# polli-labs/linnaeus

Measured on AMD Instinct MI355X. Metric: images/sec (train fwd+bwd) mFormerV1_sm 3x224x224, higher is better.
Workload: dtype bf16; 1 GPU; mFormerV1_sm train step (forward + 4-task CE loss + backward + AdamW (one HIP launch)), bf16 operands / fp32 accumulate+residual, batch 256/GPU, 3x224x224 synthetic, DropPath 0.2, gradient checkpointing off; per_gpu_batch=256, global_batch=256, parallelism=dp1, grad_mode=direct

## Files before the change

include/lnx.h:

```cpp
#ifndef LNX_H
#define LNX_H
#include <stdint.h>

#ifdef __cplusplus
extern "C" {
#endif

#define LNX_F32 0
#define LNX_BF16 1

const char* lnx_last_error(void);
int lnx_version(void);
int lnx_device_cus(void);
int lnx_set_cu_margin(int cus);

typedef struct lnx_rowmap {
    int group, pad, off;
} lnx_rowmap;

enum { LNX_ACT_NONE = 0, LNX_ACT_GELU = 1, LNX_ACT_RELU = 2, LNX_ACT_GELU_BWD = 3, LNX_ACT_RELU_BWD = 4,
       LNX_ACT_GELU_D = 5, LNX_ACT_MUL_AUX = 6 };
enum { LNX_ADDR_PLAIN = 0, LNX_ADDR_PATCH2 = 1 };

typedef struct lnx_gemm_args {
    int dtype;
    int M, N, K;
    const void* A;
    int64_t lda;
    const void* W;
    int64_t ldw;
    void* C;
    int64_t ldc;
    int out_f32;
    int a_mode, Hin, Win, Cin;
    int c_mode;
    lnx_rowmap c_map;
    const float* bias;
    void* c2;
    int64_t ldc2;
    int act;
    const void* aux;
    int64_t ldaux;
    const float* gamma;
    const float* rowscale;
    int rows_per_sample;
    const float* res;
    int64_t ldres;
    void* c8;
    int64_t ldc8;
    void* c8_scales;
} lnx_gemm_args;

int lnx_gemm_nt(const lnx_gemm_args* args, void* stream);

#define LNX_GEMM_GROUP_MAX 8
int lnx_gemm_nt_group_ok(const lnx_gemm_args* problems, int n, int accumulate);
int lnx_gemm_nt_group(const lnx_gemm_args* problems, int n, int accumulate, void* stream);

enum { LNX_NT_KERNEL_NONE = 0, LNX_NT_KERNEL_V1 = 1 , LNX_NT_KERNEL_V2 = 2 ,
       LNX_NT_KERNEL_SKINNY = 3 , LNX_NT_KERNEL_V4 = 4 ,
       LNX_NT_KERNEL_FP8 = 6 , LNX_NT_KERNEL_V7 = 7 ,
       LNX_NT_KERNEL_MX8 = 8 , LNX_NT_KERNEL_V9 = 9 ,
       LNX_NT_KERNEL_EXPERIMENT = 15 , LNX_NT_KERNEL_KINDS = 16 };
int lnx_last_nt_kernel(void);
int64_t lnx_nt_kernel_launches(int kind);
int lnx_nt_dispatch(const lnx_gemm_args* args);

int lnx_amax(const void* x, int x_dtype, int64_t ldx, int rows, int cols, float* amax, void* stream);
int lnx_quantize_fp8(const void* x, int x_dtype, int64_t ldx, int rows, int cols, const float* amax, void* y, int64_t ldy, float* scale_out, void* stream);
int lnx_gemm_nt_fp8(const lnx_gemm_args* args, const float* a_scale, const float* w_scale, void* stream);

int lnx_quantize_mxfp8(const void* x, int x_dtype, int64_t ldx, int rows, int cols, void* y, int64_t ldy, void* scales, void* stream);
int lnx_gemm_nt_mxfp8(const lnx_gemm_args* args, const void* a_scales, const void* w_scales, void* stream);

typedef struct lnx_wgrad_args {
    int dtype;
    int M, N, K;
    const void* dY;
    int64_t lddy;
    const void* A;
    int64_t lda;
    int a_mode, Hin, Win, Cin;
    float* dW;
    int64_t lddw;
    int k_perm_c;
    float* db;
    int splits;
    int k_store;
    float* ws;
    int64_t ws_floats;
    int defer;
} lnx_wgrad_args;
#define LNX_TN_WS_FLOATS (256 * (256 * 128 + 256))

int lnx_gemm_tn(const lnx_wgrad_args* args, void* stream);
int lnx_gemm_tn_flush(void* stream);
int lnx_gemm_tn_discard(void);


typedef struct lnx_ln_args {
    int M, C;
    float eps;
    const void* x;
    int x_dtype;
    int64_t ldx;
    lnx_rowmap x_map;
    const float* w;
    const float* b;
    void* y;
    int y_dtype;
    int64_t ldy;
    lnx_rowmap y_map;
    const void* add;
    int64_t ldadd;
    float* mean;
    float* rstd;
    void* y8;
    int64_t ldy8;
    void* y8_scales;
} lnx_ln_args;
int lnx_layernorm_fwd(const lnx_ln_args* args, void* stream);

typedef struct lnx_ln_bwd_args {
    int M, C;
    const void* dy;
    int dy_dtype;
    int64_t lddy;
    lnx_rowmap dy_map;
    const void* x;
    int x_dtype;
    int64_t ldx;
    lnx_rowmap x_map;
    const float* w;
    const float* mean;
    const float* rstd;
    const float* gin;
    int64_t ldgin;
    void* dx;
    int dx_dtype;
    int64_t lddx;
    float* dw;
    float* db;
    int relu_mask;
    float* ws;
    int64_t ws_floats;
    void* dx2;
    int dx2_dtype;
    int64_t lddx2;
    const float* dx2_rowscale;
    int dx2_rows_per_sample;
    void* dx2_8;
    void* dx2_8_scales;
    int64_t lddx2_8;
    int defer;
} lnx_ln_bwd_args;
int lnx_layernorm_bwd(const lnx_ln_bwd_args* args, void* stream);
int lnx_layernorm_bwd_flush(void* stream);
int lnx_layernorm_bwd_discard(void);

typedef struct lnx_dwconv_args {
    int B, H, W, C;
    const void* x;
    int x_dtype;
    const float* w49;
    const float* bias;
    int flip;
    const float* res;
    void* y;
    int y_dtype;
} lnx_dwconv_args;
int lnx_dwconv7_fwd(const lnx_dwconv_args* args, void* stream);

typedef struct lnx_dwconv_wgrad_args {
    int B, H, W, C;
    const void* x;
    int x_dtype;
    const void* dy;
    int dy_dtype;
    float* dw;
    float* db;
} lnx_dwconv_wgrad_args;
int lnx_dwconv7_wgrad(const lnx_dwconv_wgrad_args* args, void* stream);

enum { LNX_ROPE_COS = 0, LNX_ROPE_ROTATE = 1 };
int lnx_rope_cos_table(const float* freqs , int heads, int H, int W, float* cos_out ,
                       float* dsin_out ,
                       void* stream);
int lnx_rope_cos_table_hd(const float* freqs, int heads, int head_dim, int H, int W, float* cos_out, float* dsin_out, void* stream);
int lnx_rope_cossin_table_hd(const float* freqs, int heads, int head_dim, int H, int W, float* cos_out, float* sin_out, float* dsin_out, void* stream);
#define LNX_ROPE_TABLES_MAX 24
typedef struct {
    const float* freqs;
    float* cos_out;
    float* dsin_out;
    int heads, H, W;
    int head_dim;
    int rope_mode;
    float* sin_out;
} lnx_rope_table;
int lnx_rope_cos_tables(const lnx_rope_table* tables, int n, void* stream);
int64_t lnx_attn_bwd_ws_floats(int B, int N, int heads);
int64_t lnx_attn_bwd_ws_floats_hd(int B, int N, int heads, int head_dim);

typedef struct lnx_attn_args {
    int dtype;
    int B, N, E, heads;
    const void* qkv;
    const float* cos_tab;
    void* o;
    float* lse;
    const unsigned char* drop_mask;
    float drop_inv_keep;
    int head_dim;
    int rope_mode;
    const float* sin_tab;
} lnx_attn_args;
int lnx_attn_fwd(const lnx_attn_args* args, void* stream);

typedef struct lnx_attn_bwd_args {
    int dtype;
    int B, N, E, heads;
    const void* qkv;
    const float* cos_tab;
    const void* o;
    const float* lse;
    const void* d_o;
    void* dqkv;
    float* freq_ws;
    float* delta;
    const unsigned char* drop_mask;
    float drop_inv_keep;
    const float* dsin_tab;
    float* dfreqs;
    int defer_freqs;
    int head_dim;
    int rope_mode;
    const float* sin_tab;
    int grid_w;
} lnx_attn_bwd_args;
#define LNX_ATTN_DEFER_MAX 16
int lnx_attn_bwd_flush(void* stream);
int lnx_attn_bwd_discard(void);
int lnx_attn_bwd(const lnx_attn_bwd_args* args, void* stream);

enum { LNX_ATTN_KERNEL_NONE = 0, LNX_ATTN_KERNEL_RES4 = 1 , LNX_ATTN_KERNEL_RES8 = 2 ,
       LNX_ATTN_KERNEL_TILED4 = 3 , LNX_ATTN_KERNEL_TILED8 = 4  };
int lnx_attn_dispatch(int dtype, int N, int head_dim, int has_drop_mask);
int lnx_last_attn_kernel(void);

int lnx_im2col_stem(const float* x, int B, int Cin, int H, int W, void* patches, int dtype, int ldp, void* stream);

typedef struct lnx_stem_args {
    const float* x;
    const void* w;
    const float* bias;
    const float* ln_w;
    const float* ln_b;
    void* patches;
    void* pre;
    float* y;
    float* mean;
    float* rstd;
    int B, Cin, H, W, Cout;
    float eps;
} lnx_stem_args;
int lnx_stem_fwd_ok(int dtype, int Cin, int H, int W, int Cout);
int lnx_stem_fwd(const lnx_stem_args* args, void* stream);

int lnx_scale_cast(const float* in, int64_t ldin, lnx_rowmap in_map, const float* rowscale, int rows_per_sample, void* out,
                   int out_dtype, int64_t ldout, int M, int C, void* stream);

int lnx_layerscale_bwd(const float* g, const void* z, int dtype, const float* gamma, const float* rowscale,
                       int rows_per_sample, void* dz, float* dgamma, int M, int C, void* stream);

int lnx_layerscale_apply_wgrad(const float* s, const float* t, int64_t lds, const float* w, const float* b, int64_t ldw, const float* gamma, float* dw, float* db,
                               int64_t lddw, float* dgamma, int C, int K, void* stream);

int lnx_dropout_mul(void* x, int dtype, const unsigned char* mask, float inv_keep, int M, int C, void* stream);
int lnx_dropout_residual(const void* z, int z_dtype, const unsigned char* mask, float inv_keep, const float* rowscale, int rows_per_sample,
                         const float* res, float* out, int M, int C, void* stream);

int lnx_fill_rows(const float* vec, float* out, int64_t ldout, lnx_rowmap map, int M, int C, void* stream);
int lnx_colsum_rows(const float* in, int64_t ldin, lnx_rowmap map, float* out, int M, int C, void* stream);

int lnx_agg2_fwd(const float* a, const float* b, const float* w2, const float* bias1, float* out, int M, int C, void* stream);
int lnx_agg2_bwd(const float* dout, const float* a, const float* b, const float* w2, float* da, float* db_, float* dw2,
                 float* dbias1, int M, int C, void* stream);

int lnx_pack_meta(const float* meta, int width, int off, int dim, void* out, int dtype, int B, void* stream);

typedef struct lnx_meta_head_args {
    int B, C;
    int dim, off;
    const float* meta;
    int meta_width;
    float eps;
    const float* w0;
    int ldw0;
    const float *b0, *ln0_w, *ln0_b;
    const float* w1;
    int ldw1;
    const float *b1, *ln1_w, *ln1_b;
    const float* w2;
    int ldw2;
    const float *b2, *ln2_w, *ln2_b;
    float* t0;
    float *h0, *x, *h1, *n1, *h2;
    float *m0, *r0, *m1, *r1, *m2, *r2;
    float* tok;
    int64_t tok_row_stride, tok_row_offset;
} lnx_meta_head_args;
int lnx_meta_heads_supported(int C);
int lnx_meta_heads_fwd(const lnx_meta_head_args* heads, int n_heads, void* stream);

typedef struct lnx_meta_head_bwd_args {
    int B, C, dim;
    const float* g;
    int64_t g_row_stride, g_row_offset;
    const float* w1t;
    int ldw1t;
    const float* w2t;
    int ldw2t;
    const float *ln0_w, *ln1_w, *ln2_w;
    const float *t0, *h0, *x, *h1, *n1, *h2, *m0, *r0, *m1, *r1, *m2, *r2;
    float *dp2, *dp1, *dp0;
    float* part;
    float* d_w0;
    float *d_b0, *d_ln0_w, *d_ln0_b;
    float* d_w1;
    float *d_b1, *d_ln1_w, *d_ln1_b;
    float* d_w2;
    float *d_b2, *d_ln2_w, *d_ln2_b;
} lnx_meta_head_bwd_args;
int64_t lnx_meta_heads_bwd_part_floats(int B, int C);
int lnx_meta_heads_bwd(const lnx_meta_head_bwd_args* heads, int n_heads, void* stream);

enum { LNX_PREP_CAST = 0, LNX_PREP_CONV_PERM = 1, LNX_PREP_DW49 = 2 };
typedef struct lnx_prep_desc {
    const float* src;
    void* dst;
    void* dst_t;
    int rows, cols;
    int ld, ld_t;
    int P;
    int mode;
    int block_start;
} lnx_prep_desc;
int lnx_prep_weights(const lnx_prep_desc* descs_dev, int ndesc, int total_blocks, int dtype, void* stream);
int lnx_prep_blocks(int rows, int ld, int cols, int ld_t, int has_t);



typedef struct lnx_softce_args {
    int B, C;
    const float* logits;
    int64_t ld;
    const int64_t* target;
    const float* soft;
    float smoothing;
    const float* class_weight;
    int64_t ignore_index;
    const float* row_scale;
    float scale;
    float* loss;
    float* loss_sum;
    float* dlogits;
    int64_t ldd;
} lnx_softce_args;
int lnx_softce(const lnx_softce_args* args, void* stream);
#define LNX_SOFTCE_MAX_TASKS 8
int lnx_softce_multi(const lnx_softce_args* args, int n, void* stream);

typedef struct lnx_mix_args {
    const float* x;
    const int64_t* perm;
    const unsigned char* valid;
    float* out;
    int B;
    int64_t row;
    int H, W;
    float lam;
    int h0, h1, w0, w1;
    int mode;
} lnx_mix_args;
int lnx_mix_rows(const lnx_mix_args* args, void* stream);
int lnx_mix_meta(const float* aux, const unsigned char* mask, const int64_t* perm, const float* pick, const int* bounds_dev, int nchunk, int B, int D,
                 float* out_aux, unsigned char* out_mask, void* stream);

enum {
    LNX_AUG_CLAMP = 0,
    LNX_AUG_POSTERIZE = 1,
    LNX_AUG_SOLARIZE = 2,
    LNX_AUG_SOLARIZE_ADD = 3,
    LNX_AUG_INVERT = 4,
    LNX_AUG_BRIGHTNESS = 5,
    LNX_AUG_CONTRAST = 6
};
int lnx_aug_pointwise(float* x, int64_t n, int64_t per_image, int op, float p0, float p1, const float* per_image_scalar, void* stream);
int lnx_aug_saturation(float* x, int B, int64_t hw, float factor, void* stream);
int lnx_aug_rowstat(const float* x, int rows, int64_t cols, int kind, float* out, void* stream);
int lnx_aug_rescale(float* x, int64_t rows, int64_t cols, const float* minmax, void* stream);
int lnx_aug_affine(const float* x, float* y, int planes, int H, int W, const float* m6, void* stream);
int lnx_aug_stencil(const float* x, float* y, int planes, int H, int W, const float* taps_dev, int k, int mode, float ratio, void* stream);
int lnx_erase_rects(float* x, int B, int C, int H, int W, const int* rects_dev, const float* values_dev, int n_rects, void* stream);
int lnx_u8hwc_to_f32chw(const unsigned char* src, float* dst, int B, int H, int W, int C, void* stream);

#define LNX_ADAMW_MAX_GROUPS 16
typedef struct lnx_adamw_desc {
    float* p;
    float* m;
    float* v;
    const float* g;
    int64_t n;
    int group;
    int block_start;
} lnx_adamw_desc;
typedef struct lnx_adamw_hyper {
    int ngroups;
    float lr[LNX_ADAMW_MAX_GROUPS], beta1[LNX_ADAMW_MAX_GROUPS], beta2[LNX_ADAMW_MAX_GROUPS], eps[LNX_ADAMW_MAX_GROUPS],
        weight_decay[LNX_ADAMW_MAX_GROUPS];
    float bias_c1[LNX_ADAMW_MAX_GROUPS], bias_c2[LNX_ADAMW_MAX_GROUPS];
    float omb1[LNX_ADAMW_MAX_GROUPS], omb2[LNX_ADAMW_MAX_GROUPS];
} lnx_adamw_hyper;
int lnx_adamw_blocks(int64_t numel);
int lnx_grad_sumsq(const lnx_adamw_desc* descs_dev, int ndesc, int total_blocks, float* out, float* ws, void* stream);
int lnx_adamw_step(const lnx_adamw_desc* descs_dev, int ndesc, int total_blocks, const lnx_adamw_hyper* hyper, const float* sumsq, float max_norm,
                   void* stream);

typedef struct lnx_ademamix_hyper {
    int ngroups;
    float lr[LNX_ADAMW_MAX_GROUPS], beta1[LNX_ADAMW_MAX_GROUPS], beta2[LNX_ADAMW_MAX_GROUPS], eps[LNX_ADAMW_MAX_GROUPS],
        weight_decay[LNX_ADAMW_MAX_GROUPS];
    float bias_c1[LNX_ADAMW_MAX_GROUPS], bias_c2[LNX_ADAMW_MAX_GROUPS];
    float omb1[LNX_ADAMW_MAX_GROUPS], omb2[LNX_ADAMW_MAX_GROUPS];
    float alpha_t[LNX_ADAMW_MAX_GROUPS], beta3_t[LNX_ADAMW_MAX_GROUPS], omb3[LNX_ADAMW_MAX_GROUPS];
} lnx_ademamix_hyper;
int lnx_ademamix_step(const lnx_adamw_desc* descs_dev, float* const* slow_dev, int ndesc, int total_blocks, const lnx_ademamix_hyper* hyper,
                      const float* sumsq, float max_norm, void* stream);

int lnx_gradnorm_sumsq(const lnx_adamw_desc* descs_dev, int ndesc, int total_blocks, int ntasks, int64_t task_stride, float* sumsq, float* norm,
                       float* ws, void* stream);
typedef struct lnx_gradnorm_args {
    int T;
    float alpha;
    const float* norm;
    const float* loss_sum;
    const float* count;
    const float* init_loss;
    float* weights;
    float* initial_losses;
    int* initted;
    float* metrics;
} lnx_gradnorm_args;
int lnx_gradnorm_update(const lnx_gradnorm_args* args, void* stream);

enum { LNX_METRICS_CHAIN_N = 0, LNX_METRICS_CHAIN_CORRECT, LNX_METRICS_PARTIAL_N, LNX_METRICS_PARTIAL_CORRECT, LNX_METRICS_SUBSET_OOR ,
       LNX_METRICS_HEAD = 8 };
enum { LNX_METRICS_N = 0, LNX_METRICS_CORRECT1, LNX_METRICS_CORRECT3, LNX_METRICS_NULL_N, LNX_METRICS_NULL_CORRECT1, LNX_METRICS_NONNULL_N,
       LNX_METRICS_NONNULL_CORRECT1, LNX_METRICS_LOSS_N, LNX_METRICS_TASK_STRIDE = 8 };
enum { LNX_METRICS_SUM_LOSS = 0, LNX_METRICS_SUM_NULL_LOSS, LNX_METRICS_SUM_NONNULL_LOSS, LNX_METRICS_SUM_STRIDE = 4 };
#define LNX_METRICS_TASK(t) (LNX_METRICS_HEAD + LNX_METRICS_TASK_STRIDE * (t))
#define LNX_METRICS_SUBSET(n_tasks, n_bins0, s) (LNX_METRICS_TASK(n_tasks) + ((s) ? 2 * (int64_t)(n_tasks) * (n_bins0) : 0))
#define LNX_METRICS_SUM(t) (LNX_METRICS_SUM_STRIDE * (t))
typedef struct lnx_metrics_task {
    const void* logits;
    int64_t ld;
    const int64_t* target;
    const unsigned char* is_null;
    const float* loss;
    int C;
} lnx_metrics_task;
typedef struct lnx_metrics_args {
    int dtype;
    int B, n_tasks;
    lnx_metrics_task task[LNX_SOFTCE_MAX_TASKS];
    const int64_t* subset_ids[2];
    int n_bins[2];
    int64_t* counts;
    double* sums;
} lnx_metrics_args;
int lnx_metrics_table_sizes(int n_tasks, int n_bins0, int n_bins1, int64_t* n_counts, int64_t* n_sums);
int lnx_metrics_update(const lnx_metrics_args* args, void* stream);

#define LNX_PREDICT_MAX_K 16
typedef struct lnx_predict_task {
    const void* logits;
    int64_t ld;
    int C;
    const int32_t* parent;
    int null_index;
    const int64_t* id_map;
} lnx_predict_task;
typedef struct lnx_predict_args {
    int dtype;
    int B, n_tasks;
    int K;
    int consistency;
    const int32_t* k_per_sample;
    lnx_predict_task task[LNX_SOFTCE_MAX_TASKS];
    int64_t* ids;
    float* probs;
    int32_t* count;
    int32_t* flags;
} lnx_predict_args;
int lnx_predict(const lnx_predict_args* args, void* stream);

int lnx_convmlp_supported(int dtype, int C);
typedef struct lnx_convmlp_args {
    int dtype, M, C;
    const void* ln;
    const void* w1;
    const float* b1;
    const void* w2;
    const float* b2;
    const float* gamma;
    const float* rowscale;
    int rows_per_sample;
    const float* x;
    float* out;
    void* z;
    const void* y;
    const float* ln_w;
    const float* ln_b;
    float ln_eps;
    void* ln_out;
    float* mean;
    float* rstd;
} lnx_convmlp_args;
int lnx_convmlp_fwd(const lnx_convmlp_args* args, void* stream);

typedef struct lnx_convmlp_bwd_args {
    int dtype, M, C;
    const float* g;
    const void* ln;
    const void* z;
    const void* w1;
    const float* b1;
    const void* w2t;
    const void* w1t;
    const float* gamma;
    const float* rowscale;
    int rows_per_sample;
    void* act;
    void* dh;
    void* dz;
    void* dln;
    float* dgamma;
    const void* y;
    const float* ln_w;
    const float* mean;
    const float* rstd;
    float* d_ln_w;
    float* d_ln_b;
    float* ws;
    int64_t ws_floats;
    int dz_plain;
    int ln_defer;
} lnx_convmlp_bwd_args;
int lnx_convmlp_bwd(const lnx_convmlp_bwd_args* args, void* stream);
int64_t lnx_convmlp_bwd_ws_floats(int C, int M);


#define LNX_MAX_META 8
#define LNX_MAX_TASKS 16
typedef struct lnx_mformer_cfg {
    int dtype;
    int batch, img_h, img_w, in_chans;
    int dims[4];
    int conv_depths[2];
    int rope_depths[2];
    int rope_heads[2];
    int mlp_hidden[2];
    int n_meta;
    int meta_dims[LNX_MAX_META];
    int only_last_cls;
    int n_tasks;
    int task_classes[LNX_MAX_TASKS];
    int inference;
    int recompute;
    int fp8;
    int rope_mode;
} lnx_mformer_cfg;

typedef struct lnx_plan lnx_plan;
int lnx_plan_create(const lnx_mformer_cfg* cfg, lnx_plan** out);
void lnx_plan_destroy(lnx_plan* p);
int64_t lnx_plan_workspace_bytes(const lnx_plan* p);
int lnx_plan_num_params(const lnx_plan* p);
const char* lnx_plan_param_name(const lnx_plan* p, int i);
int64_t lnx_plan_param_numel(const lnx_plan* p, int i);
int lnx_plan_num_drop_calls(const lnx_plan* p);
int64_t lnx_plan_logits_numel(const lnx_plan* p);
int64_t lnx_plan_logits_offset(const lnx_plan* p, int task);
int lnx_plan_logits_ld(const lnx_plan* p, int task);
int lnx_plan_bind(lnx_plan* p, const float* const* params, float* const* grads, void* workspace);
int lnx_plan_forward(lnx_plan* p, const float* x, const float* meta, const float* drop_scales, const unsigned char* drop_mask,
                     float* feats, float* logits, void* stream);
int64_t lnx_plan_dropout_bytes(const lnx_plan* p);
int lnx_plan_set_dropout(lnx_plan* p, const unsigned char* masks, float drop_rate);
int64_t lnx_plan_attn_dropout_bytes(const lnx_plan* p);
int lnx_plan_set_attn_dropout(lnx_plan* p, const unsigned char* masks, float drop_rate);
int lnx_plan_backward(lnx_plan* p, const float* dlogits, const float* dfeats, int segment, void* stream);
int lnx_plan_backward_into(lnx_plan* p, const float* dlogits, const float* dfeats, float* const* grads, void* stream);
#define LNX_PROFILE_CLASSES 8
int lnx_plan_profile_begin(lnx_plan* p);
int lnx_plan_profile_end(lnx_plan* p, double* ms, double* work, int* launches);
#define LNX_PROFILE_CLASSES_EX 10
int lnx_plan_profile_begin_spans(lnx_plan* p);
int lnx_plan_profile_end_ex(lnx_plan* p, double* ms, double* work, double* bytes, int* launches);
int lnx_plan_set_wgrad_stream(lnx_plan* p, int on);
int lnx_plan_set_meta_stream(lnx_plan* p, int mode);
int lnx_plan_segment_params(const lnx_plan* p, int segment, int* idx_out, int max_out);

#ifdef __cplusplus
}
#endif
#endif
```

linnaeus_amd/_lib.py:

```python
from __future__ import annotations

import ctypes as C
import os

_HERE = os.path.dirname(os.path.abspath(__file__))
LIB_PATH = os.environ.get("LNX_LIB_PATH") or os.path.join(_HERE, "liblnx_hip.so")

F32, BF16 = 0, 1
ACT_NONE, ACT_GELU, ACT_RELU, ACT_GELU_BWD, ACT_RELU_BWD, ACT_GELU_D, ACT_MUL_AUX = 0, 1, 2, 3, 4, 5, 6
TN_WS_FLOATS = 256 * (256 * 128 + 256)
ADDR_PLAIN, ADDR_PATCH2 = 0, 1


class LnxError(RuntimeError):
    pass


class RowMap(C.Structure):
    _fields_ = [("group", C.c_int), ("pad", C.c_int), ("off", C.c_int)]


class GemmArgs(C.Structure):
    _fields_ = [
        ("dtype", C.c_int), ("M", C.c_int), ("N", C.c_int), ("K", C.c_int),
        ("A", C.c_void_p), ("lda", C.c_int64),
        ("W", C.c_void_p), ("ldw", C.c_int64),
        ("C", C.c_void_p), ("ldc", C.c_int64),
        ("out_f32", C.c_int),
        ("a_mode", C.c_int), ("Hin", C.c_int), ("Win", C.c_int), ("Cin", C.c_int),
        ("c_mode", C.c_int), ("c_map", RowMap),
        ("bias", C.c_void_p),
        ("c2", C.c_void_p), ("ldc2", C.c_int64),
        ("act", C.c_int),
        ("aux", C.c_void_p), ("ldaux", C.c_int64),
        ("gamma", C.c_void_p), ("rowscale", C.c_void_p), ("rows_per_sample", C.c_int),
        ("res", C.c_void_p), ("ldres", C.c_int64),
        ("c8", C.c_void_p), ("ldc8", C.c_int64), ("c8_scales", C.c_void_p),
    ]


class WgradArgs(C.Structure):
    _fields_ = [
        ("dtype", C.c_int), ("M", C.c_int), ("N", C.c_int), ("K", C.c_int),
        ("dY", C.c_void_p), ("lddy", C.c_int64),
        ("A", C.c_void_p), ("lda", C.c_int64),
        ("a_mode", C.c_int), ("Hin", C.c_int), ("Win", C.c_int), ("Cin", C.c_int),
        ("dW", C.c_void_p), ("lddw", C.c_int64),
        ("k_perm_c", C.c_int),
        ("db", C.c_void_p),
        ("splits", C.c_int),
        ("k_store", C.c_int),
        ("ws", C.c_void_p), ("ws_floats", C.c_int64),
        ("defer", C.c_int),
    ]


class SoftCEArgs(C.Structure):
    _fields_ = [
        ("B", C.c_int), ("C", C.c_int),
        ("logits", C.c_void_p), ("ld", C.c_int64),
        ("target", C.c_void_p),
        ("soft", C.c_void_p), ("smoothing", C.c_float),
        ("class_weight", C.c_void_p),
        ("ignore_index", C.c_int64),
        ("row_scale", C.c_void_p), ("scale", C.c_float),
        ("loss", C.c_void_p), ("loss_sum", C.c_void_p),
        ("dlogits", C.c_void_p), ("ldd", C.c_int64),
    ]


ADAMW_MAX_GROUPS = 16


class AdamWDesc(C.Structure):
    _fields_ = [("p", C.c_void_p), ("m", C.c_void_p), ("v", C.c_void_p), ("g", C.c_void_p), ("n", C.c_int64), ("group", C.c_int), ("block_start", C.c_int)]


class AdamWHyper(C.Structure):
    _fields_ = [("ngroups", C.c_int)] + [(k, C.c_float * ADAMW_MAX_GROUPS) for k in ("lr", "beta1", "beta2", "eps", "weight_decay", "bias_c1", "bias_c2", "omb1", "omb2")]


class AdEMAMixHyper(C.Structure):
    _fields_ = [("ngroups", C.c_int)] + [(k, C.c_float * ADAMW_MAX_GROUPS) for k in ("lr", "beta1", "beta2", "eps", "weight_decay", "bias_c1", "bias_c2", "omb1", "omb2",
                                                                                  "alpha_t", "beta3_t", "omb3")]


class GradNormArgs(C.Structure):
    _fields_ = [("T", C.c_int), ("alpha", C.c_float), ("norm", C.c_void_p), ("loss_sum", C.c_void_p), ("count", C.c_void_p), ("init_loss", C.c_void_p),
                ("weights", C.c_void_p), ("initial_losses", C.c_void_p), ("initted", C.c_void_p), ("metrics", C.c_void_p)]


METRICS_MAX_TASKS = 8
METRICS_CHAIN_N, METRICS_CHAIN_CORRECT, METRICS_PARTIAL_N, METRICS_PARTIAL_CORRECT, METRICS_SUBSET_OOR = range(5)
METRICS_HEAD = 8
METRICS_N, METRICS_CORRECT1, METRICS_CORRECT3, METRICS_NULL_N, METRICS_NULL_CORRECT1, METRICS_NONNULL_N, METRICS_NONNULL_CORRECT1, METRICS_LOSS_N = range(8)
METRICS_TASK_STRIDE = 8
METRICS_SUM_LOSS, METRICS_SUM_NULL_LOSS, METRICS_SUM_NONNULL_LOSS = range(3)
METRICS_SUM_STRIDE = 4


def metrics_task(t: int) -> int:
    return METRICS_HEAD + METRICS_TASK_STRIDE * t


def metrics_subset(n_tasks: int, n_bins0: int, s: int) -> int:
    return metrics_task(n_tasks) + (2 * n_tasks * n_bins0 if s else 0)


class MetricsTask(C.Structure):
    _fields_ = [("logits", C.c_void_p), ("ld", C.c_int64), ("target", C.c_void_p), ("is_null", C.c_void_p), ("loss", C.c_void_p), ("C", C.c_int)]


class MetricsArgs(C.Structure):
    _fields_ = [("dtype", C.c_int), ("B", C.c_int), ("n_tasks", C.c_int), ("task", MetricsTask * METRICS_MAX_TASKS),
                ("subset_ids", C.c_void_p * 2), ("n_bins", C.c_int * 2), ("counts", C.c_void_p), ("sums", C.c_void_p)]


PREDICT_MAX_K = 16


class PredictTask(C.Structure):
    _fields_ = [("logits", C.c_void_p), ("ld", C.c_int64), ("C", C.c_int), ("parent", C.c_void_p), ("null_index", C.c_int), ("id_map", C.c_void_p)]


class PredictArgs(C.Structure):
    _fields_ = [("dtype", C.c_int), ("B", C.c_int), ("n_tasks", C.c_int), ("K", C.c_int), ("consistency", C.c_int), ("k_per_sample", C.c_void_p),
                ("task", PredictTask * METRICS_MAX_TASKS), ("ids", C.c_void_p), ("probs", C.c_void_p), ("count", C.c_void_p), ("flags", C.c_void_p)]


_lib = None


def lib() -> C.CDLL:
    global _lib
    if _lib is None:
        if not os.path.exists(LIB_PATH):
            raise LnxError(
                f"{LIB_PATH} is missing: build it with `python -c 'import __graft_entry__ as g; g.build()'` "
                "(or `make -C linnaeus_amd/csrc`). linnaeus_amd has no CPU fallback."
            )
        _lib = C.CDLL(LIB_PATH)
        _lib.lnx_last_error.restype = C.c_char_p
        _lib.lnx_nt_kernel_launches.restype = C.c_int64
        _lib.lnx_convmlp_bwd_ws_floats.restype = C.c_int64
        _lib.lnx_meta_heads_bwd_part_floats.restype = C.c_int64
        if hasattr(_lib, "lnx_ademamix_step"):
            _lib.lnx_ademamix_step.argtypes = [C.c_void_p, C.c_void_p, C.c_int, C.c_int, C.POINTER(AdEMAMixHyper), C.c_void_p, C.c_float, C.c_void_p]
        if hasattr(_lib, "lnx_gradnorm_sumsq"):
            _lib.lnx_gradnorm_sumsq.argtypes = [C.c_void_p, C.c_int, C.c_int, C.c_int, C.c_int64, C.c_void_p, C.c_void_p, C.c_void_p, C.c_void_p]
        if hasattr(_lib, "lnx_metrics_update"):
            _lib.lnx_metrics_update.argtypes = [C.POINTER(MetricsArgs), C.c_void_p]
            _lib.lnx_metrics_table_sizes.argtypes = [C.c_int, C.c_int, C.c_int, C.POINTER(C.c_int64), C.POINTER(C.c_int64)]
        if hasattr(_lib, "lnx_predict"):
            _lib.lnx_predict.argtypes = [C.POINTER(PredictArgs), C.c_void_p]
            _lib.lnx_predict.restype = C.c_int
        older = bool(os.environ.get("LNX_LIB_PATH")) and os.environ.get("LNX_LIB_OLDER") == "1"
        for name in EXPORTS:
            if not hasattr(_lib, name) and not older:
                raise LnxError(f"{LIB_PATH} does not export {name}; rebuild it")
    return _lib


def check(rc: int, what: str) -> None:
    if rc != 0:
        raise LnxError(f"{what} failed (rc={rc}): {lib().lnx_last_error().decode()}")


AUG_CLAMP, AUG_POSTERIZE, AUG_SOLARIZE, AUG_SOLARIZE_ADD, AUG_INVERT, AUG_BRIGHTNESS, AUG_CONTRAST = range(7)

NT_KERNEL_NONE, NT_KERNEL_V1, NT_KERNEL_V2, NT_KERNEL_SKINNY, NT_KERNEL_V4, NT_KERNEL_FP8, NT_KERNEL_V7, NT_KERNEL_MX8, NT_KERNEL_V9, NT_KERNEL_EXPERIMENT = 0, 1, 2, 3, 4, 6, 7, 8, 9, 15

ROPE_COS, ROPE_ROTATE = 0, 1

ATTN_KERNEL_NONE, ATTN_KERNEL_RES4, ATTN_KERNEL_RES8, ATTN_KERNEL_TILED4, ATTN_KERNEL_TILED8 = range(5)

EXPORTS = [
    "lnx_last_error", "lnx_version", "lnx_device_cus", "lnx_set_cu_margin",
    "lnx_gemm_nt", "lnx_last_nt_kernel", "lnx_nt_kernel_launches", "lnx_nt_dispatch", "lnx_gemm_tn", "lnx_gemm_tn_flush", "lnx_gemm_tn_discard", "lnx_amax", "lnx_quantize_fp8", "lnx_gemm_nt_fp8", "lnx_quantize_mxfp8", "lnx_gemm_nt_mxfp8", "lnx_dropout_mul", "lnx_dropout_residual", "lnx_plan_dropout_bytes", "lnx_plan_set_dropout", "lnx_plan_attn_dropout_bytes", "lnx_plan_set_attn_dropout",
    "lnx_layernorm_fwd", "lnx_layernorm_bwd", "lnx_layernorm_bwd_flush", "lnx_layernorm_bwd_discard",
    "lnx_dwconv7_fwd", "lnx_dwconv7_wgrad",
    "lnx_gemm_nt_group_ok", "lnx_gemm_nt_group", "lnx_rope_cos_table", "lnx_rope_cos_table_hd", "lnx_rope_cossin_table_hd", "lnx_rope_cos_tables", "lnx_attn_bwd_ws_floats", "lnx_attn_bwd_ws_floats_hd", "lnx_attn_fwd", "lnx_attn_bwd", "lnx_attn_bwd_flush", "lnx_attn_bwd_discard", "lnx_attn_dispatch", "lnx_last_attn_kernel",
    "lnx_im2col_stem", "lnx_scale_cast", "lnx_layerscale_bwd", "lnx_layerscale_apply_wgrad", "lnx_fill_rows", "lnx_colsum_rows",
    "lnx_agg2_fwd", "lnx_agg2_bwd", "lnx_pack_meta", "lnx_meta_heads_supported", "lnx_meta_heads_fwd", "lnx_meta_heads_bwd", "lnx_meta_heads_bwd_part_floats", "lnx_prep_weights", "lnx_prep_blocks", "lnx_softce", "lnx_softce_multi", "lnx_stem_fwd", "lnx_stem_fwd_ok", "lnx_adamw_blocks", "lnx_grad_sumsq", "lnx_adamw_step", "lnx_ademamix_step", "lnx_gradnorm_sumsq", "lnx_gradnorm_update",
    "lnx_metrics_table_sizes", "lnx_metrics_update", "lnx_predict",
    "lnx_mix_rows", "lnx_mix_meta",
    "lnx_aug_pointwise", "lnx_aug_saturation", "lnx_aug_rowstat", "lnx_aug_rescale", "lnx_aug_affine", "lnx_aug_stencil", "lnx_erase_rects", "lnx_u8hwc_to_f32chw",
    "lnx_convmlp_supported", "lnx_convmlp_fwd", "lnx_convmlp_bwd", "lnx_convmlp_bwd_ws_floats",
    "lnx_plan_create", "lnx_plan_destroy", "lnx_plan_workspace_bytes", "lnx_plan_num_params", "lnx_plan_param_name",
    "lnx_plan_param_numel", "lnx_plan_num_drop_calls", "lnx_plan_logits_numel", "lnx_plan_logits_offset", "lnx_plan_logits_ld",
    "lnx_plan_bind", "lnx_plan_forward", "lnx_plan_backward", "lnx_plan_backward_into", "lnx_plan_segment_params", "lnx_plan_profile_begin", "lnx_plan_profile_end", "lnx_plan_profile_begin_spans", "lnx_plan_profile_end_ex", "lnx_plan_set_wgrad_stream", "lnx_plan_set_meta_stream",
]


class MetaHeadArgs(C.Structure):
    _fields_ = [
        ("B", C.c_int), ("C", C.c_int), ("dim", C.c_int), ("off", C.c_int),
        ("meta", C.c_void_p), ("meta_width", C.c_int), ("eps", C.c_float),
        ("w0", C.c_void_p), ("ldw0", C.c_int), ("b0", C.c_void_p), ("ln0_w", C.c_void_p), ("ln0_b", C.c_void_p),
        ("w1", C.c_void_p), ("ldw1", C.c_int), ("b1", C.c_void_p), ("ln1_w", C.c_void_p), ("ln1_b", C.c_void_p),
        ("w2", C.c_void_p), ("ldw2", C.c_int), ("b2", C.c_void_p), ("ln2_w", C.c_void_p), ("ln2_b", C.c_void_p),
        ("t0", C.c_void_p), ("h0", C.c_void_p), ("x", C.c_void_p), ("h1", C.c_void_p), ("n1", C.c_void_p), ("h2", C.c_void_p),
        ("m0", C.c_void_p), ("r0", C.c_void_p), ("m1", C.c_void_p), ("r1", C.c_void_p), ("m2", C.c_void_p), ("r2", C.c_void_p),
        ("tok", C.c_void_p), ("tok_row_stride", C.c_int64), ("tok_row_offset", C.c_int64),
    ]


class MetaHeadBwdArgs(C.Structure):
    _fields_ = [
        ("B", C.c_int), ("C", C.c_int), ("dim", C.c_int),
        ("g", C.c_void_p), ("g_row_stride", C.c_int64), ("g_row_offset", C.c_int64),
        ("w1t", C.c_void_p), ("ldw1t", C.c_int), ("w2t", C.c_void_p), ("ldw2t", C.c_int),
        ("ln0_w", C.c_void_p), ("ln1_w", C.c_void_p), ("ln2_w", C.c_void_p),
        ("t0", C.c_void_p), ("h0", C.c_void_p), ("x", C.c_void_p), ("h1", C.c_void_p), ("n1", C.c_void_p), ("h2", C.c_void_p),
        ("m0", C.c_void_p), ("r0", C.c_void_p), ("m1", C.c_void_p), ("r1", C.c_void_p), ("m2", C.c_void_p), ("r2", C.c_void_p),
        ("dp2", C.c_void_p), ("dp1", C.c_void_p), ("dp0", C.c_void_p), ("part", C.c_void_p),
        ("d_w0", C.c_void_p), ("d_b0", C.c_void_p), ("d_ln0_w", C.c_void_p), ("d_ln0_b", C.c_void_p),
        ("d_w1", C.c_void_p), ("d_b1", C.c_void_p), ("d_ln1_w", C.c_void_p), ("d_ln1_b", C.c_void_p),
        ("d_w2", C.c_void_p), ("d_b2", C.c_void_p), ("d_ln2_w", C.c_void_p), ("d_ln2_b", C.c_void_p),
    ]


class LnArgs(C.Structure):
    _fields_ = [
        ("M", C.c_int), ("C", C.c_int), ("eps", C.c_float),
        ("x", C.c_void_p), ("x_dtype", C.c_int), ("ldx", C.c_int64), ("x_map", RowMap),
        ("w", C.c_void_p), ("b", C.c_void_p),
        ("y", C.c_void_p), ("y_dtype", C.c_int), ("ldy", C.c_int64), ("y_map", RowMap),
        ("add", C.c_void_p), ("ldadd", C.c_int64),
        ("mean", C.c_void_p), ("rstd", C.c_void_p),
        ("y8", C.c_void_p), ("ldy8", C.c_int64), ("y8_scales", C.c_void_p),
    ]


class LnBwdArgs(C.Structure):
    _fields_ = [
        ("M", C.c_int), ("C", C.c_int),
        ("dy", C.c_void_p), ("dy_dtype", C.c_int), ("lddy", C.c_int64), ("dy_map", RowMap),
        ("x", C.c_void_p), ("x_dtype", C.c_int), ("ldx", C.c_int64), ("x_map", RowMap),
        ("w", C.c_void_p), ("mean", C.c_void_p), ("rstd", C.c_void_p),
        ("gin", C.c_void_p), ("ldgin", C.c_int64),
        ("dx", C.c_void_p), ("dx_dtype", C.c_int), ("lddx", C.c_int64),
        ("dw", C.c_void_p), ("db", C.c_void_p), ("relu_mask", C.c_int),
        ("ws", C.c_void_p), ("ws_floats", C.c_int64),
        ("dx2", C.c_void_p), ("dx2_dtype", C.c_int), ("lddx2", C.c_int64), ("dx2_rowscale", C.c_void_p), ("dx2_rows_per_sample", C.c_int),
        ("dx2_8", C.c_void_p), ("dx2_8_scales", C.c_void_p), ("lddx2_8", C.c_int64),
        ("defer", C.c_int),
    ]


class RopeTable(C.Structure):
    _fields_ = [
        ("freqs", C.c_void_p), ("cos_out", C.c_void_p), ("dsin_out", C.c_void_p),
        ("heads", C.c_int), ("H", C.c_int), ("W", C.c_int), ("head_dim", C.c_int),
        ("rope_mode", C.c_int), ("sin_out", C.c_void_p),
    ]


class DwconvArgs(C.Structure):
    _fields_ = [
        ("B", C.c_int), ("H", C.c_int), ("W", C.c_int), ("C", C.c_int),
        ("x", C.c_void_p), ("x_dtype", C.c_int), ("w49", C.c_void_p), ("bias", C.c_void_p),
        ("flip", C.c_int), ("res", C.c_void_p), ("y", C.c_void_p), ("y_dtype", C.c_int),
    ]


class DwconvWgradArgs(C.Structure):
    _fields_ = [
        ("B", C.c_int), ("H", C.c_int), ("W", C.c_int), ("C", C.c_int),
        ("x", C.c_void_p), ("x_dtype", C.c_int), ("dy", C.c_void_p), ("dy_dtype", C.c_int),
        ("dw", C.c_void_p), ("db", C.c_void_p),
    ]


class AttnArgs(C.Structure):
    _fields_ = [
        ("dtype", C.c_int), ("B", C.c_int), ("N", C.c_int), ("E", C.c_int), ("heads", C.c_int),
        ("qkv", C.c_void_p), ("cos_tab", C.c_void_p), ("o", C.c_void_p), ("lse", C.c_void_p),
        ("drop_mask", C.c_void_p), ("drop_inv_keep", C.c_float), ("head_dim", C.c_int),
        ("rope_mode", C.c_int), ("sin_tab", C.c_void_p),
    ]


class AttnBwdArgs(C.Structure):
    _fields_ = [
        ("dtype", C.c_int), ("B", C.c_int), ("N", C.c_int), ("E", C.c_int), ("heads", C.c_int),
        ("qkv", C.c_void_p), ("cos_tab", C.c_void_p), ("o", C.c_void_p), ("lse", C.c_void_p),
        ("d_o", C.c_void_p), ("dqkv", C.c_void_p), ("freq_ws", C.c_void_p), ("delta", C.c_void_p),
        ("drop_mask", C.c_void_p), ("drop_inv_keep", C.c_float),
        ("dsin_tab", C.c_void_p), ("dfreqs", C.c_void_p), ("defer_freqs", C.c_int), ("head_dim", C.c_int),
        ("rope_mode", C.c_int), ("sin_tab", C.c_void_p), ("grid_w", C.c_int),
    ]


class PrepDesc(C.Structure):
    _fields_ = [
        ("src", C.c_void_p), ("dst", C.c_void_p), ("dst_t", C.c_void_p),
        ("rows", C.c_int), ("cols", C.c_int), ("ld", C.c_int), ("ld_t", C.c_int),
        ("P", C.c_int), ("mode", C.c_int), ("block_start", C.c_int),
    ]


PREP_CAST, PREP_CONV_PERM, PREP_DW49 = 0, 1, 2


class ConvMlpArgs(C.Structure):
    _fields_ = [
        ("dtype", C.c_int), ("M", C.c_int), ("C", C.c_int),
        ("ln", C.c_void_p), ("w1", C.c_void_p), ("b1", C.c_void_p), ("w2", C.c_void_p), ("b2", C.c_void_p),
        ("gamma", C.c_void_p), ("rowscale", C.c_void_p), ("rows_per_sample", C.c_int),
        ("x", C.c_void_p), ("out", C.c_void_p), ("z", C.c_void_p),
        ("y", C.c_void_p), ("ln_w", C.c_void_p), ("ln_b", C.c_void_p), ("ln_eps", C.c_float), ("ln_out", C.c_void_p),
        ("mean", C.c_void_p), ("rstd", C.c_void_p),
    ]


class ConvMlpBwdArgs(C.Structure):
    _fields_ = [
        ("dtype", C.c_int), ("M", C.c_int), ("C", C.c_int),
        ("g", C.c_void_p), ("ln", C.c_void_p), ("z", C.c_void_p), ("w1", C.c_void_p), ("b1", C.c_void_p),
        ("w2t", C.c_void_p), ("w1t", C.c_void_p), ("gamma", C.c_void_p), ("rowscale", C.c_void_p), ("rows_per_sample", C.c_int),
        ("act", C.c_void_p), ("dh", C.c_void_p), ("dz", C.c_void_p), ("dln", C.c_void_p), ("dgamma", C.c_void_p),
        ("y", C.c_void_p), ("ln_w", C.c_void_p), ("mean", C.c_void_p), ("rstd", C.c_void_p), ("d_ln_w", C.c_void_p), ("d_ln_b", C.c_void_p),
        ("ws", C.c_void_p), ("ws_floats", C.c_int64),
        ("dz_plain", C.c_int), ("ln_defer", C.c_int),
    ]


class StemArgs(C.Structure):
    _fields_ = [("x", C.c_void_p), ("w", C.c_void_p), ("bias", C.c_void_p), ("ln_w", C.c_void_p), ("ln_b", C.c_void_p), ("patches", C.c_void_p),
                ("pre", C.c_void_p), ("y", C.c_void_p), ("mean", C.c_void_p), ("rstd", C.c_void_p), ("B", C.c_int), ("Cin", C.c_int), ("H", C.c_int),
                ("W", C.c_int), ("Cout", C.c_int), ("eps", C.c_float)]


class MixArgs(C.Structure):
    _fields_ = [
        ("x", C.c_void_p), ("perm", C.c_void_p), ("valid", C.c_void_p), ("out", C.c_void_p),
        ("B", C.c_int), ("row", C.c_int64), ("H", C.c_int), ("W", C.c_int), ("lam", C.c_float),
        ("h0", C.c_int), ("h1", C.c_int), ("w0", C.c_int), ("w1", C.c_int), ("mode", C.c_int),
    ]
```

linnaeus_amd/csrc/convmlp.hip:

```cpp
#include <stdlib.h>

#include "common.hpp"
#include "../../include/lnx.h"

namespace {

struct CmP {
    const unsigned char* ln;
    const unsigned char* w1;
    const unsigned char* w2;
    const unsigned char* w2t;
    const unsigned char* w1t;
    const unsigned char* zin;
    const float* b1;
    const float* b2;
    const float* gamma;
    const float* rowscale;
    const float* x;
    const float* g;
    float* out;
    unsigned char* z;
    unsigned char* act;
    unsigned char* dh;
    unsigned char* dz;
    unsigned char* dln;
    float* dgamma;
    int M, C, rps;
    const unsigned char* y;
    const float* lnw;
    const float* lnb;
    float eps;
    unsigned char* ln_out;
    float* mean;
    float* rstd;
    float* part;
    int64_t part_floats;
    int ln_defer;
    int tile_slot;
    int dz_plain;
    float* dlnw;
    float* dlnb;
};

__device__ __forceinline__ void mfma16(f32x4_t& acc, const uint4& a, const uint4& b) {
    acc = __builtin_amdgcn_mfma_f32_16x16x32_bf16(__builtin_bit_cast(bf16x8_t, a), __builtin_bit_cast(bf16x8_t, b), acc, 0, 0, 0);
}

__device__ __forceinline__ int key4(int a) { return (4 - (a & 3)) & 3; }

#define CM_DS_READ128(dst, addr, OFF) asm volatile("ds_read_b128 %0, %1 offset:" #OFF : "=v"(dst) : "v"(addr) : "memory")

template <int NK> struct Geo {
    static constexpr int C = 32 * NK;
    static constexpr int PART = NK * 4096;
    static constexpr int CT = C / 16;
};

template <int NK, int NW>
__device__ __forceinline__ void dma_nmajor(unsigned char* lds_part, const unsigned char* W, int n0, int wave, int lane) {
    constexpr int C = Geo<NK>::C;
    constexpr int NINS = 4 * NK;
    static_assert(NINS % NW == 0, "DMA pieces must divide evenly over the waves");
#pragma unroll
    for (int t = 0; t < NINS / NW; ++t) {
        const int i = wave + NW * t;
        const int ks = i >> 2, rb = i & 3;
        const int row = 16 * rb + (lane >> 2), u = lane & 3;
        const unsigned char* src = W + ((int64_t)(n0 + row) * C + ks * 32 + ((u ^ key4(row >> 3)) << 3)) * 2;
        __builtin_amdgcn_global_load_lds((const __attribute__((address_space(1))) void*)src,
                                         (__attribute__((address_space(3))) void*)(lds_part + i * 1024), 16, 0, 0);
    }
}

template <int NK, int NW>
__device__ __forceinline__ void dma_cmajor(unsigned char* lds_part, const unsigned char* W, int n0, int wave, int lane) {
    constexpr int C = Geo<NK>::C;
    constexpr int RB = C / 16;
    constexpr int NINS = 2 * RB;
#pragma unroll
    for (int t = 0; t < NINS / NW; ++t) {
        const int i = wave + NW * t;
        const int ks2 = i / RB, rb = i % RB;
        const int row = 16 * rb + (lane >> 2), u = lane & 3;
        const unsigned char* src = W + ((int64_t)row * (4 * C) + n0 + ks2 * 32 + ((u ^ key4(row >> 2)) << 3)) * 2;
        __builtin_amdgcn_global_load_lds((const __attribute__((address_space(1))) void*)src,
                                         (__attribute__((address_space(3))) void*)(lds_part + i * 1024), 16, 0, 0);
    }
}

template <int NK, int MT>
__device__ __forceinline__ void prod_nmajor(f32x4_t (&h)[4][MT], uint32_t part_addr, int s, int g, const uint4 (&xf)[MT][NK]) {
    const uint32_t unit = (uint32_t)((g ^ key4(s >> 2)) << 4);
    const uint32_t base = part_addr + (uint32_t)((8 * (s >> 2) + (s & 3)) * 64) + unit;
#pragma unroll
    for (int nt = 0; nt < 4; ++nt)
#pragma unroll
        for (int mt = 0; mt < MT; ++mt) h[nt][mt] = f32x4_t{0.f, 0.f, 0.f, 0.f};
#pragma unroll
    for (int ks = 0; ks < NK; ++ks) {
        uint4 wf[4];
        const uint32_t a = base + ks * 4096;
        CM_DS_READ128(wf[0], a, 0);
        CM_DS_READ128(wf[1], a, 256);
        CM_DS_READ128(wf[2], a, 2048);
        CM_DS_READ128(wf[3], a, 2304);
        asm volatile("s_waitcnt lgkmcnt(0)" ::: "memory");
        __builtin_amdgcn_sched_barrier(0);
#pragma unroll
        for (int nt = 0; nt < 4; ++nt)
#pragma unroll
            for (int mt = 0; mt < MT; ++mt) mfma16(h[nt][mt], wf[nt], xf[mt][ks]);
    }
}

template <int NK, int MT, int KB>
__device__ __forceinline__ void prod_nmajor_b(f32x4_t (&h)[4][MT], uint32_t part_addr, int s, int g, const uint4 (&xf)[MT][NK]) {
    const uint32_t unit = (uint32_t)((g ^ key4(s >> 2)) << 4);
    const uint32_t base = part_addr + (uint32_t)((8 * (s >> 2) + (s & 3)) * 64) + unit;
#pragma unroll
    for (int nt = 0; nt < 4; ++nt)
#pragma unroll
        for (int mt = 0; mt < MT; ++mt) h[nt][mt] = f32x4_t{0.f, 0.f, 0.f, 0.f};
#pragma unroll
    for (int k0 = 0; k0 < NK; k0 += KB) {
        uint4 wf[KB][4];
#pragma unroll
        for (int kb = 0; kb < KB; ++kb) {
            if (k0 + kb < NK) {
                const uint32_t a = base + (k0 + kb) * 4096;
                CM_DS_READ128(wf[kb][0], a, 0);
                CM_DS_READ128(wf[kb][1], a, 256);
                CM_DS_READ128(wf[kb][2], a, 2048);
                CM_DS_READ128(wf[kb][3], a, 2304);
            }
        }
        asm volatile("s_waitcnt lgkmcnt(0)" ::: "memory");
        __builtin_amdgcn_sched_barrier(0);
#pragma unroll
        for (int kb = 0; kb < KB; ++kb) {
            if (k0 + kb < NK) {
#pragma unroll
                for (int nt = 0; nt < 4; ++nt)
#pragma unroll
                    for (int mt = 0; mt < MT; ++mt) mfma16(h[nt][mt], wf[kb][nt], xf[mt][k0 + kb]);
            }
        }
    }
}

template <int NK, int MT>
__device__ __forceinline__ void prod_cmajor(f32x4_t (&o)[Geo<NK>::CT][MT], uint32_t part_addr, int s, int g, const uint4 (&pf)[MT][2]) {
    constexpr int C = Geo<NK>::C;
    constexpr int CT = Geo<NK>::CT;
    const uint32_t base = part_addr + (uint32_t)(s * 64) + (uint32_t)((g ^ key4(s >> 2)) << 4);
    constexpr int GB = CT % 6 == 0 ? 6 : (CT % 4 == 0 ? 4 : CT);
#pragma unroll
    for (int ks2 = 0; ks2 < 2; ++ks2) {
#pragma unroll
        for (int c0 = 0; c0 < CT; c0 += GB) {
            uint4 wf[GB];
#pragma unroll
            for (int b = 0; b < GB; ++b) {
                const uint32_t a = base + (uint32_t)(ks2 * C * 64 + (c0 + b) * 1024);
                CM_DS_READ128(wf[b], a, 0);
            }
            asm volatile("s_waitcnt lgkmcnt(0)" ::: "memory");
            __builtin_amdgcn_sched_barrier(0);
#pragma unroll
            for (int b = 0; b < GB; ++b)
#pragma unroll
                for (int mt = 0; mt < MT; ++mt) mfma16(o[c0 + b][mt], wf[b], pf[mt][ks2]);
        }
    }
}

template <int NK, int MT>
__device__ __forceinline__ void prod_nmajor_pipe(f32x4_t (&h)[4][MT], uint32_t part_addr, int s, int g, const uint4 (&xf)[MT][NK]) {
    const uint32_t unit = (uint32_t)((g ^ key4(s >> 2)) << 4);
    const uint32_t base = part_addr + (uint32_t)((8 * (s >> 2) + (s & 3)) * 64) + unit;
#pragma unroll
    for (int nt = 0; nt < 4; ++nt)
#pragma unroll
        for (int mt = 0; mt < MT; ++mt) h[nt][mt] = f32x4_t{0.f, 0.f, 0.f, 0.f};
    uint4 wf[2][4];
    CM_DS_READ128(wf[0][0], base, 0);
    CM_DS_READ128(wf[0][1], base, 256);
    CM_DS_READ128(wf[0][2], base, 2048);
    CM_DS_READ128(wf[0][3], base, 2304);
#pragma unroll
    for (int ks = 0; ks < NK; ++ks) {
        if (ks + 1 < NK) {
            const uint32_t a = base + (ks + 1) * 4096;
            CM_DS_READ128(wf[(ks + 1) & 1][0], a, 0);
            CM_DS_READ128(wf[(ks + 1) & 1][1], a, 256);
            CM_DS_READ128(wf[(ks + 1) & 1][2], a, 2048);
            CM_DS_READ128(wf[(ks + 1) & 1][3], a, 2304);
            asm volatile("s_waitcnt lgkmcnt(4)" ::: "memory");
        } else {
            asm volatile("s_waitcnt lgkmcnt(0)" ::: "memory");
        }
        __builtin_amdgcn_sched_barrier(0);
#pragma unroll
        for (int nt = 0; nt < 4; ++nt)
#pragma unroll
            for (int mt = 0; mt < MT; ++mt) mfma16(h[nt][mt], wf[ks & 1][nt], xf[mt][ks]);
    }
}

template <int NK, int MT>
__device__ __forceinline__ void prod_cmajor_pipe(f32x4_t (&o)[Geo<NK>::CT][MT], uint32_t part_addr, int s, int g, const uint4 (&pf)[MT][2]) {
    constexpr int C = Geo<NK>::C;
    constexpr int CT = Geo<NK>::CT;
    const uint32_t base = part_addr + (uint32_t)(s * 64) + (uint32_t)((g ^ key4(s >> 2)) << 4);
    constexpr int GB = 4;
    constexpr int NB = 2 * CT / GB;
    static_assert(CT % GB == 0, "channel tiles must split into batches of 4");
    uint4 wf[2][GB];
#pragma unroll
    for (int b = 0; b < GB; ++b) CM_DS_READ128(wf[0][b], base + (uint32_t)(b * 1024), 0);
#pragma unroll
    for (int bt = 0; bt < NB; ++bt) {
        const int ks2 = (bt * GB) / CT, c0 = (bt * GB) % CT;
        if (bt + 1 < NB) {
            const int ks2n = ((bt + 1) * GB) / CT, c0n = ((bt + 1) * GB) % CT;
#pragma unroll
            for (int b = 0; b < GB; ++b) CM_DS_READ128(wf[(bt + 1) & 1][b], base + (uint32_t)(ks2n * C * 64 + (c0n + b) * 1024), 0);
            asm volatile("s_waitcnt lgkmcnt(4)" ::: "memory");
        } else {
            asm volatile("s_waitcnt lgkmcnt(0)" ::: "memory");
        }
        __builtin_amdgcn_sched_barrier(0);
#pragma unroll
        for (int b = 0; b < GB; ++b)
#pragma unroll
            for (int mt = 0; mt < MT; ++mt) mfma16(o[c0 + b][mt], wf[bt & 1][b], pf[mt][ks2]);
    }
}

__device__ __forceinline__ uint4 pack8(const f32x4_t& lo, const f32x4_t& hi) {
    Vec16<bf16_t> v;
#pragma unroll
    for (int j = 0; j < 4; ++j) {
        v.set(j, lo[j]);
        v.set(4 + j, hi[j]);
    }
    return v.raw;
}

__device__ __forceinline__ float g_sum(float v) {
    v += __shfl_xor(v, 16, 64);
    v += __shfl_xor(v, 32, 64);
    return v;
}
template <int CTRL> __device__ __forceinline__ float dpp_get(float v) {
    return __builtin_bit_cast(float, __builtin_amdgcn_update_dpp(0, __builtin_bit_cast(int, v), CTRL, 0xf, 0xf, false));
}
__device__ __forceinline__ float row16_sum(float v) {
    v += dpp_get<0xB1>(v);
    v += dpp_get<0x4E>(v);
    v += dpp_get<0x141>(v);
    v += dpp_get<0x140>(v);
    return v;
}
template <int NK>
__device__ __forceinline__ void ln_row_frags(uint4 (&xf)[NK], const float* w, const float* b, int g, float eps, float& mu, float& rs) {
    constexpr float invC = 1.0f / (float)Geo<NK>::C;
    float v[NK][8];
    float sum = 0.f;
#pragma unroll
    for (int ks = 0; ks < NK; ++ks) {
        Vec16<bf16_t> t;
        t.raw = xf[ks];
#pragma unroll
        for (int j = 0; j < 8; ++j) v[ks][j] = t.get(j);
        sum += ((v[ks][0] + v[ks][1]) + (v[ks][2] + v[ks][3])) + ((v[ks][4] + v[ks][5]) + (v[ks][6] + v[ks][7]));
    }
    mu = g_sum(sum) * invC;
    float sq = 0.f;
#pragma unroll
    for (int ks = 0; ks < NK; ++ks)
#pragma unroll
        for (int j = 0; j < 8; ++j) {
            v[ks][j] -= mu;
            sq = fmaf(v[ks][j], v[ks][j], sq);
        }
    rs = 1.0f / sqrtf(fmaf(g_sum(sq), invC, eps));
#pragma unroll
    for (int ks = 0; ks < NK; ++ks) {
        const int c = ks * 32 + 8 * g;
        const float4 w0 = *reinterpret_cast<const float4*>(w + c), w1 = *reinterpret_cast<const float4*>(w + c + 4);
        const float4 b0 = *reinterpret_cast<const float4*>(b + c), b1 = *reinterpret_cast<const float4*>(b + c + 4);
        const float wv[8] = {w0.x, w0.y, w0.z, w0.w, w1.x, w1.y, w1.z, w1.w};
        const float bv[8] = {b0.x, b0.y, b0.z, b0.w, b1.x, b1.y, b1.z, b1.w};
        Vec16<bf16_t> o;
#pragma unroll
        for (int j = 0; j < 8; ++j) o.set(j, fmaf(v[ks][j] * rs, wv[j], bv[j]));
        xf[ks] = o.raw;
    }
}
template <int NK>
struct LnRow {
    uint2 yr[Geo<NK>::CT];
    float mu, rs;
};
template <int NK>
__device__ __forceinline__ void ln_bwd_fetch(LnRow<NK>& r, const CmP& p, int m, int g) {
    constexpr int C = Geo<NK>::C;
    const int mc = m < p.M ? m : p.M - 1;
#pragma unroll
    for (int ct = 0; ct < Geo<NK>::CT; ++ct) r.yr[ct] = *reinterpret_cast<const uint2*>(p.y + ((int64_t)mc * C + ct * 16 + 4 * g) * 2);
    r.mu = p.mean[mc];
    r.rs = p.rstd[mc];
}
template <int NK, int MT, int MTI>
__device__ __forceinline__ void ln_bwd_rows(const CmP& p, const f32x4_t (&dl)[Geo<NK>::CT][MT], const LnRow<NK>& row, int m, int s, int g, const float* lnws,
                                            float* dls) {
    constexpr int C = Geo<NK>::C;
    constexpr int CT = Geo<NK>::CT;
    constexpr float invC = 1.0f / (float)C;
    const bool mv = m < p.M;
    const int mc = mv ? m : p.M - 1;
    const uint2 (&yr)[CT] = row.yr;
    const float mu = row.mu, rs = row.rs;
    float xh[CT][4], gv[CT][4];
    float s1 = 0.f, s2 = 0.f;
#pragma unroll
    for (int ct = 0; ct < CT; ++ct) {
        const int c = ct * 16 + 4 * g;
        const float4 w4 = *reinterpret_cast<const float4*>(lnws + c);
        const float wv[4] = {w4.x, w4.y, w4.z, w4.w};
        const bf16_t* yh = reinterpret_cast<const bf16_t*>(&yr[ct]);
#pragma unroll
        for (int r = 0; r < 4; ++r) {
            const float d = (float)(bf16_t)dl[ct][MTI][r];
            const float x = ((float)yh[r] - mu) * rs;
            xh[ct][r] = x;
            gv[ct][r] = d * wv[r];
            s1 += gv[ct][r];
            s2 = fmaf(gv[ct][r], x, s2);
            const float dm = mv ? d : 0.f;
            const float a = row16_sum(dm * x), b = row16_sum(dm);
            if (s == 0) {
                atomicAdd(&dls[c + r], a);
                atomicAdd(&dls[C + c + r], b);
            }
        }
    }
    const float m1 = g_sum(s1) * invC, m2 = g_sum(s2) * invC;
#pragma unroll
    for (int ct = 0; ct < CT; ++ct) {
        uint2 v;
        bf16_t* vh = reinterpret_cast<bf16_t*>(&v);
#pragma unroll
        for (int r = 0; r < 4; ++r) vh[r] = (bf16_t)(rs * (gv[ct][r] - m1 - xh[ct][r] * m2));
        *reinterpret_cast<uint2*>(p.dln + ((int64_t)mc * C + ct * 16 + 4 * g) * 2) = v;
    }
}

#ifdef CM_STAMP
__device__ unsigned long long g_cm_stamp[8];
#define CM_T(i) do { __builtin_amdgcn_sched_barrier(0); unsigned long long t_; asm volatile("s_memtime %0\n\ts_waitcnt lgkmcnt(0)" : "=s"(t_) :: "memory"); \
                     __builtin_amdgcn_sched_barrier(0); tsum[i] += t_ - tlast; tlast = t_; } while (0)
#else
#define CM_T(i) do { } while (0)
#endif

template <int NK, int MT, int NW, bool LNF>
__global__ __launch_bounds__(64 * NW) void convmlp_fwd_kernel(const CmP p) {
#ifdef CM_STAMP
    unsigned long long tsum[8] = {0, 0, 0, 0, 0, 0, 0, 0}, tlast;
    asm volatile("s_memtime %0\n\ts_waitcnt lgkmcnt(0)" : "=s"(tlast)::"memory");
#endif
    constexpr int C = Geo<NK>::C;
    constexpr int CT = Geo<NK>::CT;
    constexpr int PART = Geo<NK>::PART;
    constexpr int STAGE = 2 * PART;
    constexpr int NCH = 4 * C / 64;
    constexpr int NLD = 8 * NK / NW;
    extern __shared__ __attribute__((aligned(16))) unsigned char smem[];
    float* b1s = reinterpret_cast<float*>(smem + 3 * STAGE);

    const int lane = threadIdx.x & 63;
    const int wave = __builtin_amdgcn_readfirstlane(threadIdx.x >> 6);
    const int s = lane & 15, g = lane >> 4;
    const int m_base = blockIdx.x * (16 * NW * MT) + wave * (16 * MT);
    const uint32_t lds0 = (uint32_t)(uintptr_t)(__attribute__((address_space(3))) unsigned char*)smem;

    for (int i = threadIdx.x; i < 4 * C; i += 64 * NW) b1s[i] = p.b1[i];

    uint4 xf[MT][NK];
#pragma unroll
    for (int mt = 0; mt < MT; ++mt) {
        int m = m_base + mt * 16 + s;
        if (m >= p.M) m = p.M - 1;
#pragma unroll
        for (int ks = 0; ks < NK; ++ks) xf[mt][ks] = ld16((LNF ? p.y : p.ln) + ((int64_t)m * C + ks * 32 + 8 * g) * 2);
    }
    if constexpr (LNF) {
#pragma unroll
        for (int mt = 0; mt < MT; ++mt) {
            float mu, rs;
            ln_row_frags<NK>(xf[mt], p.lnw, p.lnb, g, p.eps, mu, rs);
            const int m = m_base + mt * 16 + s;
            if (m < p.M) {
                if (p.ln_out) {
#pragma unroll
                    for (int ks = 0; ks < NK; ++ks) st16(p.ln_out + ((int64_t)m * C + ks * 32 + 8 * g) * 2, xf[mt][ks]);
                }
                if (p.mean && g == 0) {
                    p.mean[m] = mu;
                    p.rstd[m] = rs;
                }
            }
        }
    }
    f32x4_t o[CT][MT];
#pragma unroll
    for (int ct = 0; ct < CT; ++ct)
#pragma unroll
        for (int mt = 0; mt < MT; ++mt) o[ct][mt] = f32x4_t{0.f, 0.f, 0.f, 0.f};

    __syncthreads();
    dma_nmajor<NK, NW>(smem, p.w1, 0, wave, lane);
    dma_cmajor<NK, NW>(smem + PART, p.w2, 0, wave, lane);
    dma_nmajor<NK, NW>(smem + STAGE, p.w1, 64, wave, lane);
    dma_cmajor<NK, NW>(smem + STAGE + PART, p.w2, 64, wave, lane);
    CM_T(0);
    for (int j = 0; j < NCH; ++j) {
        const int stg = j % 3;
        if (j + 1 < NCH) asm volatile("s_waitcnt vmcnt(%0)" ::"n"(NLD) : "memory");
        else asm volatile("s_waitcnt vmcnt(0)" ::: "memory");
        CM_T(1);
        __builtin_amdgcn_s_barrier();
        CM_T(2);
        if (j + 2 < NCH) {
            unsigned char* nx = smem + ((j + 2) % 3) * STAGE;
            dma_nmajor<NK, NW>(nx, p.w1, 64 * (j + 2), wave, lane);
            dma_cmajor<NK, NW>(nx + PART, p.w2, 64 * (j + 2), wave, lane);
        }
        const uint32_t st = lds0 + stg * STAGE;
        f32x4_t h[4][MT];
        CM_T(3);
        prod_nmajor_pipe<NK, MT>(h, st, s, g, xf);
        CM_T(4);
        uint4 pf[MT][2];
        {
            f32x4_t bv[4];
            const uint32_t ba = lds0 + 3 * STAGE + (uint32_t)((64 * j + 8 * g) * 4);
            CM_DS_READ128(bv[0], ba, 0);
            CM_DS_READ128(bv[1], ba, 16);
            CM_DS_READ128(bv[2], ba, 128);
            CM_DS_READ128(bv[3], ba, 144);
            asm volatile("s_waitcnt lgkmcnt(0)" ::: "memory");
            __builtin_amdgcn_sched_barrier(0);
#pragma unroll
            for (int mt = 0; mt < MT; ++mt)
#pragma unroll
                for (int n2 = 0; n2 < 4; n2 += 2) {
                    f32x4_t hv[2] = {h[n2][mt], h[n2 + 1][mt]};
                    gelu4_bias_n<2>(hv, &bv[n2]);
                    h[n2][mt] = hv[0];
                    h[n2 + 1][mt] = hv[1];
                }
#pragma unroll
            for (int mt = 0; mt < MT; ++mt) {
                pf[mt][0] = pack8(h[0][mt], h[1][mt]);
                pf[mt][1] = pack8(h[2][mt], h[3][mt]);
            }
        }
        CM_T(5);
        prod_cmajor_pipe<NK, MT>(o, st + PART, s, g, pf);
        CM_T(6);
    }
#pragma unroll
    for (int mt = 0; mt < MT; ++mt) {
        const int m = m_base + mt * 16 + s;
        if (m >= p.M) continue;
        const float rs = p.rowscale ? p.rowscale[m / p.rps] : 1.0f;
        float4 xrv[CT], b2v[CT], gmv[CT];
#pragma unroll
        for (int ct = 0; ct < CT; ++ct) {
            const int c = ct * 16 + 4 * g;
            xrv[ct] = *reinterpret_cast<const float4*>(p.x + (int64_t)m * C + c);
            b2v[ct] = *reinterpret_cast<const float4*>(p.b2 + c);
            gmv[ct] = *reinterpret_cast<const float4*>(p.gamma + c);
        }
#pragma unroll
        for (int ct = 0; ct < CT; ++ct) {
            const int c = ct * 16 + 4 * g;
            const float4 b2 = b2v[ct], gm = gmv[ct], xr = xrv[ct];
            const float z0 = o[ct][mt][0] + b2.x, z1 = o[ct][mt][1] + b2.y, z2 = o[ct][mt][2] + b2.z, z3 = o[ct][mt][3] + b2.w;
            if (p.z) {
                uint2 zz;
                bf16_t* zh = reinterpret_cast<bf16_t*>(&zz);
                zh[0] = (bf16_t)z0; zh[1] = (bf16_t)z1; zh[2] = (bf16_t)z2; zh[3] = (bf16_t)z3;
                *reinterpret_cast<uint2*>(p.z + ((int64_t)m * C + c) * 2) = zz;
            }
            *reinterpret_cast<float4*>(p.out + (int64_t)m * C + c) =
                make_float4(xr.x + rs * gm.x * z0, xr.y + rs * gm.y * z1, xr.z + rs * gm.z * z2, xr.w + rs * gm.w * z3);
        }
    }
    CM_T(7);
#ifdef CM_STAMP
    if (blockIdx.x == gridDim.x / 2 && threadIdx.x == 0)
        for (int i = 0; i < 8; ++i) g_cm_stamp[i] = tsum[i];
#endif
}
#ifdef CM_STAMP
extern "C" int lnx_dbg_convmlp_stamps(unsigned long long* out8) { return (int)hipMemcpyFromSymbol(out8, HIP_SYMBOL(g_cm_stamp), 64); }
#endif

template <int NK, int MT, int NW, bool ST, bool LNB, bool DG>
__global__ __launch_bounds__(64 * NW) void convmlp_bwd_kernel(const CmP p) {
    constexpr int C = Geo<NK>::C;
    constexpr int CT = Geo<NK>::CT;
    constexpr int PART = Geo<NK>::PART;
    constexpr int STAGE = 3 * PART;
    constexpr int NCH = 4 * C / 64;
    constexpr int NLD = 12 * NK / NW;
    extern __shared__ __attribute__((aligned(16))) unsigned char smem[];
    float* b1s = reinterpret_cast<float*>(smem + 2 * STAGE);
    float* dgs = b1s + 4 * C;
    float* lws = dgs + C;
    float* dls = lws + C;

    const int lane = threadIdx.x & 63;
    const int wave = __builtin_amdgcn_readfirstlane(threadIdx.x >> 6);
    const int s = lane & 15, g = lane >> 4;
    const int m_base = blockIdx.x * (16 * NW * MT) + wave * (16 * MT);
    const uint32_t lds0 = (uint32_t)(uintptr_t)(__attribute__((address_space(3))) unsigned char*)smem;

    for (int i = threadIdx.x; i < 4 * C; i += 64 * NW) b1s[i] = p.b1[i];
    for (int i = threadIdx.x; i < C; i += 64 * NW) {
        dgs[i] = 0.f;
        if constexpr (LNB) {
            lws[i] = p.lnw[i];
            dls[i] = dls[C + i] = 0.f;
        }
    }
    __syncthreads();

    uint4 xf[MT][NK], zf[MT][NK];
    bool mvalid[MT];
#pragma unroll
    for (int mt = 0; mt < MT; ++mt) {
        int m = m_base + mt * 16 + s;
        mvalid[mt] = m < p.M;
        if (!mvalid[mt]) m = p.M - 1;
        const float rs = p.rowscale ? p.rowscale[m / p.rps] : 1.0f;
        float4 g0v[NK], g1v[NK], a0v[NK], a1v[NK];
        uint4 zraw[NK];
#pragma unroll
        for (int ks = 0; ks < NK; ++ks) {
            const int c = ks * 32 + 8 * g;
            xf[mt][ks] = ld16(p.ln + ((int64_t)m * C + c) * 2);
            g0v[ks] = *reinterpret_cast<const float4*>(p.g + (int64_t)m * C + c);
            g1v[ks] = *reinterpret_cast<const float4*>(p.g + (int64_t)m * C + c + 4);
            a0v[ks] = *reinterpret_cast<const float4*>(p.gamma + c);
            a1v[ks] = *reinterpret_cast<const float4*>(p.gamma + c + 4);
            if constexpr (DG) zraw[ks] = ld16(p.zin + ((int64_t)m * C + c) * 2);
        }
#pragma unroll
        for (int ks = 0; ks < NK; ++ks) {
            const int c = ks * 32 + 8 * g;
            const float4 g0 = g0v[ks], g1 = g1v[ks], a0 = a0v[ks], a1 = a1v[ks];
            Vec16<bf16_t> zin, dzv, dzs;
            if constexpr (DG) zin.raw = zraw[ks];
            const float gv[8] = {g0.x, g0.y, g0.z, g0.w, g1.x, g1.y, g1.z, g1.w};
            const float av[8] = {a0.x, a0.y, a0.z, a0.w, a1.x, a1.y, a1.z, a1.w};
#pragma unroll
            for (int j = 0; j < 8; ++j) {
                const float sg = rs * gv[j];
                dzv.set(j, sg * av[j]);
                dzs.set(j, p.dz_plain ? sg : sg * av[j]);
                if constexpr (DG) {
                    const float dgp = mvalid[mt] ? sg * zin.get(j) : 0.f;
                    float t = dgp;
                    t += __shfl_xor(t, 1, 64);
                    t += __shfl_xor(t, 2, 64);
                    t += __shfl_xor(t, 4, 64);
                    t += __shfl_xor(t, 8, 64);
                    if (s == 0) atomicAdd(&dgs[c + j], t);
                }
            }
            zf[mt][ks] = dzv.raw;
            st16(p.dz + ((int64_t)m * C + c) * 2, dzs.raw);
        }
    }
    f32x4_t dl[CT][MT];
#pragma unroll
    for (int ct = 0; ct < CT; ++ct)
#pragma unroll
        for (int mt = 0; mt < MT; ++mt) dl[ct][mt] = f32x4_t{0.f, 0.f, 0.f, 0.f};
    LnRow<NK> lrow;
    if constexpr (LNB) ln_bwd_fetch<NK>(lrow, p, m_base + s, g);

    __syncthreads();
    dma_nmajor<NK, NW>(smem, p.w1, 0, wave, lane);
    dma_nmajor<NK, NW>(smem + PART, p.w2t, 0, wave, lane);
    dma_cmajor<NK, NW>(smem + 2 * PART, p.w1t, 0, wave, lane);
    for (int j = 0; j < NCH; ++j) {
        const int stg = j & 1;
        __builtin_amdgcn_s_barrier();
        if (j + 1 < NCH) {
            unsigned char* nx = smem + (stg ^ 1) * STAGE;
            dma_nmajor<NK, NW>(nx, p.w1, 64 * (j + 1), wave, lane);
            dma_nmajor<NK, NW>(nx + PART, p.w2t, 64 * (j + 1), wave, lane);
            dma_cmajor<NK, NW>(nx + 2 * PART, p.w1t, 64 * (j + 1), wave, lane);
            asm volatile("s_waitcnt vmcnt(%0)" ::"n"(NLD) : "memory");
        } else {
            asm volatile("s_waitcnt vmcnt(0)" ::: "memory");
        }
        __builtin_amdgcn_s_barrier();
        const uint32_t st = lds0 + stg * STAGE;
        f32x4_t h[4][MT], da[4][MT];
        prod_nmajor_pipe<NK, MT>(h, st, s, g, xf);
        prod_nmajor_pipe<NK, MT>(da, st + PART, s, g, zf);
        f32x4_t bv[4];
        const uint32_t ba = lds0 + 2 * STAGE + (uint32_t)((64 * j + 8 * g) * 4);
        CM_DS_READ128(bv[0], ba, 0);
        CM_DS_READ128(bv[1], ba, 16);
        CM_DS_READ128(bv[2], ba, 128);
        CM_DS_READ128(bv[3], ba, 144);
        asm volatile("s_waitcnt lgkmcnt(0)" ::: "memory");
        __builtin_amdgcn_sched_barrier(0);
#pragma unroll
        for (int mt = 0; mt < MT; ++mt)
#pragma unroll
            for (int n2 = 0; n2 < 4; n2 += 2) {
                f32x4_t hv[2] = {h[n2][mt], h[n2 + 1][mt]}, dv[2] = {da[n2][mt], da[n2 + 1][mt]};
                gelu4_bias_grad_n<2>(hv, &bv[n2], dv);
                h[n2][mt] = hv[0];
                h[n2 + 1][mt] = hv[1];
                da[n2][mt] = dv[0];
                da[n2 + 1][mt] = dv[1];
            }
        uint4 pa[MT][2], pd[MT][2];
#pragma unroll
        for (int mt = 0; mt < MT; ++mt) {
            pa[mt][0] = pack8(h[0][mt], h[1][mt]);
            pa[mt][1] = pack8(h[2][mt], h[3][mt]);
            pd[mt][0] = pack8(da[0][mt], da[1][mt]);
            pd[mt][1] = pack8(da[2][mt], da[3][mt]);
            const int m = min(m_base + mt * 16 + s, p.M - 1);
            if constexpr (ST) {
                const int64_t off = ((int64_t)m * (4 * C) + 64 * j + 8 * g) * 2;
                st16(p.act + off, pa[mt][0]);
                st16(p.act + off + 64, pa[mt][1]);
                st16(p.dh + off, pd[mt][0]);
                st16(p.dh + off + 64, pd[mt][1]);
            }
        }
        prod_cmajor_pipe<NK, MT>(dl, st + 2 * PART, s, g, pd);
    }
    if constexpr (LNB) {
        static_assert(MT == 1, "ln_bwd_rows is instantiated per m-tile");
        ln_bwd_rows<NK, MT, 0>(p, dl, lrow, m_base + s, s, g, lws, dls);
    } else {
#pragma unroll
        for (int mt = 0; mt < MT; ++mt) {
            const int m = min(m_base + mt * 16 + s, p.M - 1);
#pragma unroll
            for (int ct = 0; ct < CT; ++ct) {
                const int c = ct * 16 + 4 * g;
                uint2 v;
                bf16_t* vh = reinterpret_cast<bf16_t*>(&v);
                vh[0] = (bf16_t)dl[ct][mt][0]; vh[1] = (bf16_t)dl[ct][mt][1]; vh[2] = (bf16_t)dl[ct][mt][2]; vh[3] = (bf16_t)dl[ct][mt][3];
                *reinterpret_cast<uint2*>(p.dln + ((int64_t)m * C + c) * 2) = v;
            }
        }
    }
    __syncthreads();
    if constexpr (DG)
        for (int i = threadIdx.x; i < C; i += 64 * NW) atomicAdd(p.dgamma + i, dgs[i]);
    if constexpr (LNB)
        for (int i = threadIdx.x; i < 2 * C; i += 64 * NW) p.part[(int64_t)blockIdx.x * (2 * C) + i] = dls[i];
}


template <int NK>
__device__ __forceinline__ void dma_all_nmajor(unsigned char* img, const unsigned char* W, int wave, int lane) {
    constexpr int C = Geo<NK>::C;
    constexpr int NCH = 4 * C / 64;
    constexpr int NINS = 4 * NK;
    for (int q = wave; q < NCH * NINS; q += 8) {
        const int j = q / NINS, i = q % NINS;
        const int ks = i >> 2, rb = i & 3;
        const int row = 16 * rb + (lane >> 2), u = lane & 3;
        const unsigned char* src = W + ((int64_t)(64 * j + row) * C + ks * 32 + ((u ^ key4(row >> 3)) << 3)) * 2;
        __builtin_amdgcn_global_load_lds((const __attribute__((address_space(1))) void*)src,
                                         (__attribute__((address_space(3))) void*)(img + j * Geo<NK>::PART + i * 1024), 16, 0, 0);
    }
}
template <int NK>
__device__ __forceinline__ void dma_all_cmajor(unsigned char* img, const unsigned char* W, int wave, int lane) {
    constexpr int C = Geo<NK>::C;
    constexpr int NCH = 4 * C / 64;
    constexpr int RB = C / 16;
    constexpr int NINS = 2 * RB;
    for (int q = wave; q < NCH * NINS; q += 8) {
        const int j = q / NINS, i = q % NINS;
        const int ks2 = i / RB, rb = i % RB;
        const int row = 16 * rb + (lane >> 2), u = lane & 3;
        const unsigned char* src = W + ((int64_t)row * (4 * C) + 64 * j + ks2 * 32 + ((u ^ key4(row >> 2)) << 3)) * 2;
        __builtin_amdgcn_global_load_lds((const __attribute__((address_space(1))) void*)src,
                                         (__attribute__((address_space(3))) void*)(img + j * Geo<NK>::PART + i * 1024), 16, 0, 0);
    }
}

typedef __attribute__((ext_vector_type(4))) short cm_s16x4;
template <int NK, int MT>
__device__ __forceinline__ void prod_tr_nmajor(f32x4_t (&o)[Geo<NK>::CT][MT], uint32_t part_addr, int s, int g, const uint4 (&pf)[MT][2]) {
    constexpr int CT = Geo<NK>::CT;
    const int q = s >> 2, pp = s & 3;
#pragma unroll
    for (int ks2 = 0; ks2 < 2; ++ks2) {
        const int n = 32 * ks2 + 8 * g + q;
        uint2 lo[CT], hi[CT];
#pragma unroll
        for (int ct = 0; ct < CT; ++ct) {
            const int ks = ct >> 1;
            const int unit = 2 * (ct & 1) + (pp >> 1);
            const uint32_t a = part_addr + (uint32_t)(ks * 4096 + n * 64 + ((unit ^ key4(g)) << 4) + (pp & 1) * 8);
            asm volatile("ds_read_b64_tr_b16 %0, %1" : "=v"(lo[ct]) : "v"(a) : "memory");
            asm volatile("ds_read_b64_tr_b16 %0, %1 offset:256" : "=v"(hi[ct]) : "v"(a) : "memory");
        }
        asm volatile("s_waitcnt lgkmcnt(0)" ::: "memory");
        __builtin_amdgcn_sched_barrier(0);
#pragma unroll
        for (int ct = 0; ct < CT; ++ct) {
            const uint4 wf = make_uint4(lo[ct].x, lo[ct].y, hi[ct].x, hi[ct].y);
#pragma unroll
            for (int mt = 0; mt < MT; ++mt) mfma16(o[ct][mt], wf, pf[mt][ks2]);
        }
    }
}

template <bool V> struct BoolC { static constexpr bool value = V; };
template <int NK, bool LNF, int SAVE>
__global__ __launch_bounds__(512) void convmlp_fwd_res_kernel(const CmP p) {
    constexpr int MT = 2;
    constexpr int C = Geo<NK>::C;
    constexpr int CT = Geo<NK>::CT;
    constexpr int PART = Geo<NK>::PART;
    constexpr int NCH = 4 * C / 64;
    extern __shared__ __attribute__((aligned(16))) unsigned char smem[];
    unsigned char* w1img = smem;
    unsigned char* w2img = smem + NCH * PART;
    float* b1s = reinterpret_cast<float*>(smem + 2 * NCH * PART);
    float* b2s = b1s + 4 * C;
    float* gms = b2s + C;
    float* lws = gms + C;
    float* lbs = lws + C;
    const int lane = threadIdx.x & 63;
    const int wave = __builtin_amdgcn_readfirstlane(threadIdx.x >> 6);
    const int s = lane & 15, g = lane >> 4;
    const uint32_t lds0 = (uint32_t)(uintptr_t)(__attribute__((address_space(3))) unsigned char*)smem;

    for (int i = threadIdx.x; i < 4 * C; i += 512) b1s[i] = p.b1[i];
    for (int i = threadIdx.x; i < C; i += 512) {
        b2s[i] = p.b2[i];
        gms[i] = p.gamma[i];
        if constexpr (LNF) {
            lws[i] = p.lnw[i];
            lbs[i] = p.lnb[i];
        }
    }
    const bool dyn = p.tile_slot >= 0;
    const TileShare sh = tile_share((p.M + 31) / 32);
    unsigned* const ctr = &g_tile_ctr[dyn ? p.tile_slot : 0][sh.part][0];
    int drawn = dyn ? sched_draw_counted(ctr) : 0;
    dma_all_nmajor<NK>(w1img, p.w1, wave, lane);
    dma_all_cmajor<NK>(w2img, p.w2, wave, lane);
    asm volatile("s_waitcnt vmcnt(0)" ::: "memory");
    __syncthreads();

    const int ntile = (p.M + 31) / 32;
    auto load_x = [&](uint4 (&dst)[MT][NK], int tile) __attribute__((always_inline)) {
#pragma unroll
        for (int mt = 0; mt < MT; ++mt) {
            const int m = min(tile * 32 + mt * 16 + s, p.M - 1);
#pragma unroll
            for (int ks = 0; ks < NK; ++ks) dst[mt][ks] = ld16((LNF ? p.y : p.ln) + ((int64_t)m * C + ks * 32 + 8 * g) * 2);
        }
    };
    const int xbase = sh.base, xcnt = sh.cnt, xwaves = 8 * sh.workers;
    const int last_draw = xcnt + xwaves - 1;
    int pos = dyn ? __builtin_amdgcn_readfirstlane(drawn) : sh.index * 8 + wave;
    bool reset_ctr = dyn && pos == last_draw;
    uint4 xf[MT][NK];
    if (pos < xcnt) load_x(xf, xbase + pos);
    const float* rsp = p.rowscale ? p.rowscale : p.gamma;
    const float rsf = p.rowscale ? 1.0f : 0.0f;

    int next = 0;
    for (; pos < xcnt; pos = next) {
        const int tile = xbase + pos;
        const int m_base = tile * 32;
        if constexpr (LNF) {
#pragma unroll
            for (int mt = 0; mt < MT; ++mt) {
                float mu, rs;
                ln_row_frags<NK>(xf[mt], lws, lbs, g, p.eps, mu, rs);
                const int m = min(m_base + mt * 16 + s, p.M - 1);
                if constexpr (SAVE != 0) {
#pragma unroll
                    for (int ks = 0; ks < NK; ++ks) st16(p.ln_out + ((int64_t)m * C + ks * 32 + 8 * g) * 2, xf[mt][ks]);
                    if (g == 0) {
                        p.mean[m] = mu;
                        p.rstd[m] = rs;
                    }
                }
            }
        }
        if constexpr (LNF) __builtin_amdgcn_sched_barrier(0);
        if (dyn) drawn = sched_draw_counted(ctr);
        float4 xrv[MT][CT];
        float rsv[MT];
        f32x4_t o[CT][MT];
#pragma unroll
        for (int ct = 0; ct < CT; ++ct)
#pragma unroll
            for (int mt = 0; mt < MT; ++mt) o[ct][mt] = f32x4_t{0.f, 0.f, 0.f, 0.f};
        auto chunk = [&](const int j, auto lastc) __attribute__((always_inline)) {
            constexpr bool LAST = decltype(lastc)::value;
            if constexpr (LAST) {
                __builtin_amdgcn_sched_barrier(0);
                if (dyn) {
                    next = __builtin_amdgcn_readfirstlane(drawn);
                    reset_ctr = reset_ctr || next == last_draw;
                } else {
                    next = pos + xwaves;
                }
#pragma unroll
                for (int mt = 0; mt < MT; ++mt) {
                    const int m = min(m_base + mt * 16 + s, p.M - 1);
#pragma unroll
                    for (int ct = 0; ct < CT; ++ct) xrv[mt][ct] = *reinterpret_cast<const float4*>(p.x + (int64_t)m * C + ct * 16 + 4 * g);
                    rsv[mt] = rsp[p.rowscale ? m / p.rps : 0];
                }
            }
            f32x4_t h[4][MT];
            prod_nmajor_b<NK, MT, NK>(h, lds0 + j * PART, s, g, xf);
            if constexpr (LAST) {
                __builtin_amdgcn_sched_barrier(0);
                load_x(xf, next < xcnt ? xbase + next : tile);
            }
            f32x4_t bv[4];
            const uint32_t ba = lds0 + 2 * NCH * PART + (uint32_t)((64 * j + 8 * g) * 4);
            CM_DS_READ128(bv[0], ba, 0);
            CM_DS_READ128(bv[1], ba, 16);
            CM_DS_READ128(bv[2], ba, 128);
            CM_DS_READ128(bv[3], ba, 144);
            asm volatile("s_waitcnt lgkmcnt(0)" ::: "memory");
            __builtin_amdgcn_sched_barrier(0);
            constexpr int GK = NK == 3 ? 1 : 2;
#pragma unroll
            for (int mt = 0; mt < MT; ++mt)
#pragma unroll
                for (int n2 = 0; n2 < 4; n2 += GK) {
                    f32x4_t hv[GK];
#pragma unroll
                    for (int k = 0; k < GK; ++k) hv[k] = h[n2 + k][mt];
                    gelu4_bias_n<GK>(hv, &bv[n2]);
#pragma unroll
                    for (int k = 0; k < GK; ++k) h[n2 + k][mt] = hv[k];
                }
            uint4 pf[MT][2];
#pragma unroll
            for (int mt = 0; mt < MT; ++mt) {
                pf[mt][0] = pack8(h[0][mt], h[1][mt]);
                pf[mt][1] = pack8(h[2][mt], h[3][mt]);
            }
            prod_cmajor<NK, MT>(o, lds0 + NCH * PART + j * PART, s, g, pf);
        };
#pragma unroll 1
        for (int j = 0; j < NCH - 1; ++j) chunk(j, BoolC<false>{});
        chunk(NCH - 1, BoolC<true>{});
#pragma unroll
        for (int mt = 0; mt < MT; ++mt) {
            const int m = min(m_base + mt * 16 + s, p.M - 1);
            const float rs = fmaf(rsv[mt] - 1.0f, rsf, 1.0f);
#pragma unroll
            for (int ct = 0; ct < CT; ++ct) {
                const int c = ct * 16 + 4 * g;
                const float4 b2 = *reinterpret_cast<const float4*>(b2s + c);
                const float4 gm = *reinterpret_cast<const float4*>(gms + c);
                const float4 xr = xrv[mt][ct];
                const float z0 = o[ct][mt][0] + b2.x, z1 = o[ct][mt][1] + b2.y, z2 = o[ct][mt][2] + b2.z, z3 = o[ct][mt][3] + b2.w;
                if constexpr (SAVE == 1) {
                    uint2 zz;
                    bf16_t* zh = reinterpret_cast<bf16_t*>(&zz);
                    zh[0] = (bf16_t)z0; zh[1] = (bf16_t)z1; zh[2] = (bf16_t)z2; zh[3] = (bf16_t)z3;
                    *reinterpret_cast<uint2*>(p.z + ((int64_t)m * C + c) * 2) = zz;
                }
                *reinterpret_cast<float4*>(p.out + (int64_t)m * C + c) =
                    make_float4(xr.x + rs * gm.x * z0, xr.y + rs * gm.y * z1, xr.z + rs * gm.z * z2, xr.w + rs * gm.w * z3);
            }
        }
    }
    if (reset_ctr && lane == 0) sched_reset(ctr);
}

template <int NK, int MT, bool ST, bool LNB, bool DG>
__global__ __launch_bounds__(512) void convmlp_bwd_res_kernel(const CmP p) {
    constexpr int C = Geo<NK>::C;
    constexpr int CT = Geo<NK>::CT;
    constexpr int PART = Geo<NK>::PART;
    constexpr int NCH = 4 * C / 64;
    extern __shared__ __attribute__((aligned(16))) unsigned char smem[];
    unsigned char* w1img = smem;
    unsigned char* w2timg = smem + NCH * PART;
    float* b1s = reinterpret_cast<float*>(smem + 2 * NCH * PART);
    float* dgs = b1s + 4 * C;
    float* lws = dgs + C;
    float* dls = lws + C;
    float* gms = dls + 2 * C;
    const int lane = threadIdx.x & 63;
    const int wave = __builtin_amdgcn_readfirstlane(threadIdx.x >> 6);
    const int s = lane & 15, g = lane >> 4;
    const uint32_t lds0 = (uint32_t)(uintptr_t)(__attribute__((address_space(3))) unsigned char*)smem;

    for (int i = threadIdx.x; i < 4 * C; i += 512) b1s[i] = p.b1[i];
    for (int i = threadIdx.x; i < C; i += 512) {
        dgs[i] = 0.f;
        gms[i] = p.gamma[i];
        if constexpr (LNB) {
            lws[i] = p.lnw[i];
            dls[i] = dls[C + i] = 0.f;
        }
    }
    const bool dyn = p.tile_slot >= 0;
    const TileShare sh = tile_share((p.M + 16 * MT - 1) / (16 * MT));
    unsigned* const ctr = &g_tile_ctr[dyn ? p.tile_slot : 0][sh.part][0];
    int drawn = dyn ? sched_draw_counted(ctr) : 0;
    dma_all_nmajor<NK>(w1img, p.w1, wave, lane);
    dma_all_nmajor<NK>(w2timg, p.w2t, wave, lane);
    asm volatile("s_waitcnt vmcnt(0)" ::: "memory");
    __syncthreads();

    float dgp[NK][8];
#pragma unroll
    for (int ks = 0; ks < NK; ++ks)
#pragma unroll
        for (int j = 0; j < 8; ++j) dgp[ks][j] = 0.f;

    const int ntile = (p.M + 16 * MT - 1) / (16 * MT);
    const float* rsp = p.rowscale ? p.rowscale : p.gamma;
    const float rsf = p.rowscale ? 1.0f : 0.0f;
    struct TileIn {
        uint4 x[MT][NK], z[MT][NK];
        float4 g0[MT][NK], g1[MT][NK];
        float rs[MT];
        LnRow<NK> lr[MT];
    };
    auto fetch_tile = [&](TileIn& t, int tile) __attribute__((always_inline)) {
#pragma unroll
        for (int mt = 0; mt < MT; ++mt) {
            const int m = min(tile * (16 * MT) + mt * 16 + s, p.M - 1);
#pragma unroll
            for (int ks = 0; ks < NK; ++ks) {
                const int c = ks * 32 + 8 * g;
                t.x[mt][ks] = ld16(p.ln + ((int64_t)m * C + c) * 2);
                t.g0[mt][ks] = *reinterpret_cast<const float4*>(p.g + (int64_t)m * C + c);
                t.g1[mt][ks] = *reinterpret_cast<const float4*>(p.g + (int64_t)m * C + c + 4);
                if constexpr (DG) t.z[mt][ks] = ld16(p.zin + ((int64_t)m * C + c) * 2);
            }
            t.rs[mt] = rsp[p.rowscale ? m / p.rps : 0];
            if constexpr (LNB) ln_bwd_fetch<NK>(t.lr[mt], p, m, g);
        }
    };
    const int xbase = sh.base, xcnt = sh.cnt, xwaves = 8 * sh.workers;
    const int last_draw = xcnt + xwaves - 1;
    int pos = dyn ? __builtin_amdgcn_readfirstlane(drawn) : sh.index * 8 + wave;
    bool reset_ctr = dyn && pos == last_draw;
    TileIn cur;
    if (pos < xcnt) fetch_tile(cur, xbase + pos);
    int next = 0;
    for (; pos < xcnt; pos = next) {
        const int tile = xbase + pos;
        const int m_base = tile * (16 * MT);
        uint4 xf[MT][NK], zf[MT][NK];
        LnRow<NK> lrow[MT];
#pragma unroll
        for (int mt = 0; mt < MT; ++mt) {
            int m = m_base + mt * 16 + s;
            const bool mv = m < p.M;
            if (!mv) m = p.M - 1;
            const float rs = fmaf(cur.rs[mt] - 1.0f, rsf, 1.0f);
            lrow[mt] = cur.lr[mt];
#pragma unroll
            for (int ks = 0; ks < NK; ++ks) {
                const int c = ks * 32 + 8 * g;
                xf[mt][ks] = cur.x[mt][ks];
                const float4 g0 = cur.g0[mt][ks], g1 = cur.g1[mt][ks];
                const float4 a0 = *reinterpret_cast<const float4*>(gms + c), a1 = *reinterpret_cast<const float4*>(gms + c + 4);
                Vec16<bf16_t> zin, dzv, dzs;
                if constexpr (DG) zin.raw = cur.z[mt][ks];
                const float gv[8] = {g0.x, g0.y, g0.z, g0.w, g1.x, g1.y, g1.z, g1.w};
                const float av[8] = {a0.x, a0.y, a0.z, a0.w, a1.x, a1.y, a1.z, a1.w};
#pragma unroll
                for (int j = 0; j < 8; ++j) {
                    const float sg = rs * gv[j];
                    dzv.set(j, sg * av[j]);
                    dzs.set(j, p.dz_plain ? sg : sg * av[j]);
                    if constexpr (DG) dgp[ks][j] = fmaf(mv ? sg : 0.f, zin.get(j), dgp[ks][j]);
                }
                zf[mt][ks] = dzv.raw;
                st16(p.dz + ((int64_t)m * C + c) * 2, dzs.raw);
            }
        }
        if (dyn) drawn = sched_draw_counted(ctr);
        f32x4_t dl[CT][MT];
#pragma unroll
        for (int ct = 0; ct < CT; ++ct)
#pragma unroll
            for (int mt = 0; mt < MT; ++mt) dl[ct][mt] = f32x4_t{0.f, 0.f, 0.f, 0.f};
#pragma unroll 1
        for (int j = 0; j < NCH; ++j) {
            f32x4_t h[4][MT], da[4][MT];
            prod_nmajor_b<NK, MT, NK>(h, lds0 + j * PART, s, g, xf);
            prod_nmajor_b<NK, MT, NK>(da, lds0 + NCH * PART + j * PART, s, g, zf);
            f32x4_t bv[4];
            const uint32_t ba = lds0 + 2 * NCH * PART + (uint32_t)((64 * j + 8 * g) * 4);
            CM_DS_READ128(bv[0], ba, 0);
            CM_DS_READ128(bv[1], ba, 16);
            CM_DS_READ128(bv[2], ba, 128);
            CM_DS_READ128(bv[3], ba, 144);
            asm volatile("s_waitcnt lgkmcnt(0)" ::: "memory");
            __builtin_amdgcn_sched_barrier(0);
#pragma unroll
            for (int mt = 0; mt < MT; ++mt)
#pragma unroll
                for (int n2 = 0; n2 < 4; n2 += 2) {
                    f32x4_t hv[2] = {h[n2][mt], h[n2 + 1][mt]}, dv[2] = {da[n2][mt], da[n2 + 1][mt]};
                    gelu4_bias_grad_n<2>(hv, &bv[n2], dv);
                    h[n2][mt] = hv[0];
                    h[n2 + 1][mt] = hv[1];
                    da[n2][mt] = dv[0];
                    da[n2 + 1][mt] = dv[1];
                }
            uint4 pd[MT][2];
#pragma unroll
            for (int mt = 0; mt < MT; ++mt) {
                const uint4 pa0 = pack8(h[0][mt], h[1][mt]), pa1 = pack8(h[2][mt], h[3][mt]);
                pd[mt][0] = pack8(da[0][mt], da[1][mt]);
                pd[mt][1] = pack8(da[2][mt], da[3][mt]);
                const int m = min(m_base + mt * 16 + s, p.M - 1);
                if constexpr (ST) {
                    const int64_t off = ((int64_t)m * (4 * C) + 64 * j + 8 * g) * 2;
                    st16(p.act + off, pa0);
                    st16(p.act + off + 64, pa1);
                    st16(p.dh + off, pd[mt][0]);
                    st16(p.dh + off + 64, pd[mt][1]);
                }
            }
            prod_tr_nmajor<NK, MT>(dl, lds0 + j * PART, s, g, pd);
        }
        __builtin_amdgcn_sched_barrier(0);
        if (dyn) {
            next = __builtin_amdgcn_readfirstlane(drawn);
            reset_ctr = reset_ctr || next == last_draw;
        } else {
            next = pos + xwaves;
        }
        fetch_tile(cur, next < xcnt ? xbase + next : tile);
        if constexpr (LNB) {
            ln_bwd_rows<NK, MT, 0>(p, dl, lrow[0], m_base + s, s, g, lws, dls);
            if constexpr (MT == 2) ln_bwd_rows<NK, MT, 1>(p, dl, lrow[MT - 1], m_base + 16 + s, s, g, lws, dls);
        } else {
#pragma unroll
            for (int mt = 0; mt < MT; ++mt) {
                const int m = min(m_base + mt * 16 + s, p.M - 1);
#pragma unroll
                for (int ct = 0; ct < CT; ++ct) {
                    const int c = ct * 16 + 4 * g;
                    uint2 v;
                    bf16_t* vh = reinterpret_cast<bf16_t*>(&v);
                    vh[0] = (bf16_t)dl[ct][mt][0]; vh[1] = (bf16_t)dl[ct][mt][1]; vh[2] = (bf16_t)dl[ct][mt][2]; vh[3] = (bf16_t)dl[ct][mt][3];
                    *reinterpret_cast<uint2*>(p.dln + ((int64_t)m * C + c) * 2) = v;
                }
            }
        }
    }
    if constexpr (DG) {
#pragma unroll
        for (int ks = 0; ks < NK; ++ks)
#pragma unroll
            for (int j = 0; j < 8; ++j) {
                float t = dgp[ks][j];
                t += __shfl_xor(t, 1, 64);
                t += __shfl_xor(t, 2, 64);
                t += __shfl_xor(t, 4, 64);
                t += __shfl_xor(t, 8, 64);
                if (s == 0) atomicAdd(&dgs[ks * 32 + 8 * g + j], t);
            }
    }
    __syncthreads();
    if constexpr (DG)
        for (int i = threadIdx.x; i < C; i += 512) atomicAdd(p.dgamma + i, dgs[i]);
    if constexpr (LNB)
        for (int i = threadIdx.x; i < 2 * C; i += 512) p.part[(int64_t)blockIdx.x * (2 * C) + i] = dls[i];
    if (reset_ctr && lane == 0) sched_reset(ctr);
}

__global__ __launch_bounds__(256) void ln_partials_reduce_kernel(const float* __restrict__ part, int nwg, int C, float* __restrict__ dw, float* __restrict__ db) {
    const int e = blockIdx.x * 256 + threadIdx.x;
    if (e >= 2 * C) return;
    const int per = (nwg + gridDim.y - 1) / gridDim.y;
    const int w0 = blockIdx.y * per, w1 = min(nwg, w0 + per);
    float t0 = 0.f, t1 = 0.f, t2 = 0.f, t3 = 0.f;
    int w = w0;
    for (; w + 4 <= w1; w += 4) {
        t0 += part[(int64_t)w * 2 * C + e];
        t1 += part[(int64_t)(w + 1) * 2 * C + e];
        t2 += part[(int64_t)(w + 2) * 2 * C + e];
        t3 += part[(int64_t)(w + 3) * 2 * C + e];
    }
    for (; w < w1; ++w) t0 += part[(int64_t)w * 2 * C + e];
    const float t = (t0 + t1) + (t2 + t3);
    if (w0 < w1) atomicAdd((e < C ? dw : db) + (e < C ? e : e - C), t);
}

static const bool nw8 = !(getenv("LNX_CM_NW") && atoi(getenv("LNX_CM_NW")) == 4);

static int bwd_grid(int C, int M) {
    if (C <= 96) {
        const int rows = C == 32 ? 32 : 16;
        const int grid = cdiv(cdiv(M, rows), 8);
        return grid > 256 ? 256 : grid;
    }
    return cdiv(M, 16 * (nw8 ? 8 : 4));
}

static int res_room() {
    const int cus = device_cus();
    const int room = persistent_cus(cus > 0 ? cus : 256);
    return room > 256 ? 256 : room;
}

template <int NK, bool LNF, int SAVE>
int launch_fwd_res_t(const CmP& p, hipStream_t st) {
    const size_t lds = 2 * (4 * Geo<NK>::C / 64) * Geo<NK>::PART + 8 * Geo<NK>::C * sizeof(float);
    static bool attr = false;
    if (!attr) {
        (void)hipFuncSetAttribute(reinterpret_cast<const void*>(&convmlp_fwd_res_kernel<NK, LNF, SAVE>), hipFuncAttributeMaxDynamicSharedMemorySize, (int)lds);
        attr = true;
    }
    int grid = cdiv(cdiv(p.M, 32), 8);
    const int room = res_room();
    if (grid > room) grid = room;
    CmP q = p;
    q.tile_slot = tile_sched_static() ? -1 : tile_slot_of(st);
    hipLaunchKernelGGL((convmlp_fwd_res_kernel<NK, LNF, SAVE>), dim3(grid), dim3(512), lds, st, q);
    return 0;
}
template <int NK>
int launch_fwd_res(const CmP& p, hipStream_t st) {
    if (p.y) return p.z ? launch_fwd_res_t<NK, true, 1>(p, st) : (p.ln_out ? launch_fwd_res_t<NK, true, 2>(p, st) : launch_fwd_res_t<NK, true, 0>(p, st));
    return p.z ? launch_fwd_res_t<NK, false, 1>(p, st) : launch_fwd_res_t<NK, false, 0>(p, st);
}
inline int reduce_ln_partials(const CmP& p, int nwg, hipStream_t st) {
    if (p.ln_defer) {
        ln_postpone_reduce(p.part, nwg, p.C, p.dlnw, p.dlnb, nwg >= 64 ? 64 : 1, st);
        return 0;
    }
    hipLaunchKernelGGL(ln_partials_reduce_kernel, dim3(cdiv(2 * p.C, 256), nwg >= 64 ? 64 : 1), dim3(256), 0, st, p.part, nwg, p.C, p.dlnw, p.dlnb);
    return 0;
}
template <int NK, int MT, bool ST, bool LNB, bool DG>
int launch_bwd_res_t(const CmP& p, hipStream_t st) {
    const size_t lds = 2 * (4 * Geo<NK>::C / 64) * Geo<NK>::PART + 9 * Geo<NK>::C * sizeof(float);
    static bool attr = false;
    if (!attr) {
        (void)hipFuncSetAttribute(reinterpret_cast<const void*>(&convmlp_bwd_res_kernel<NK, MT, ST, LNB, DG>), hipFuncAttributeMaxDynamicSharedMemorySize, (int)lds);
        attr = true;
    }
    int grid = bwd_grid(p.C, p.M);
    if (LNB && (int64_t)grid * 2 * p.C > p.part_floats) return -1;
    const int room = res_room();
    if (grid > room) grid = room;
    CmP q = p;
    q.tile_slot = tile_sched_static() ? -1 : tile_slot_of(st);
    hipLaunchKernelGGL((convmlp_bwd_res_kernel<NK, MT, ST, LNB, DG>), dim3(grid), dim3(512), lds, st, q);
    return LNB ? reduce_ln_partials(p, grid, st) : 0;
}
template <int NK, int MT>
int launch_bwd_res(const CmP& p, hipStream_t st) {
    if (p.zin == nullptr) {
        if (p.y) return p.act ? launch_bwd_res_t<NK, MT, true, true, false>(p, st) : launch_bwd_res_t<NK, MT, false, true, false>(p, st);
        return p.act ? launch_bwd_res_t<NK, MT, true, false, false>(p, st) : launch_bwd_res_t<NK, MT, false, false, false>(p, st);
    }
    if (p.y) return p.act ? launch_bwd_res_t<NK, MT, true, true, true>(p, st) : launch_bwd_res_t<NK, MT, false, true, true>(p, st);
    return p.act ? launch_bwd_res_t<NK, MT, true, false, true>(p, st) : launch_bwd_res_t<NK, MT, false, false, true>(p, st);
}

template <int NK, int MT, int NW, bool LNF>
int launch_fwd_t(const CmP& p, hipStream_t st) {
    const size_t lds = 3 * 2 * Geo<NK>::PART + 4 * Geo<NK>::C * sizeof(float);
    static bool attr = false;
    if (!attr) {
        (void)hipFuncSetAttribute(reinterpret_cast<const void*>(&convmlp_fwd_kernel<NK, MT, NW, LNF>), hipFuncAttributeMaxDynamicSharedMemorySize, (int)lds);
        attr = true;
    }
    hipLaunchKernelGGL((convmlp_fwd_kernel<NK, MT, NW, LNF>), dim3(cdiv(p.M, 16 * NW * MT)), dim3(64 * NW), lds, st, p);
    return 0;
}
template <int NK, int MT, int NW>
int launch_fwd(const CmP& p, hipStream_t st) {
    return p.y ? launch_fwd_t<NK, MT, NW, true>(p, st) : launch_fwd_t<NK, MT, NW, false>(p, st);
}

template <int NK, int MT, int NW, bool ST, bool LNB, bool DG>
int launch_bwd_t(const CmP& p, hipStream_t st) {
    const size_t lds = 2 * 3 * Geo<NK>::PART + 8 * Geo<NK>::C * sizeof(float);
    static bool attr = false;
    if (!attr) {
        (void)hipFuncSetAttribute(reinterpret_cast<const void*>(&convmlp_bwd_kernel<NK, MT, NW, ST, LNB, DG>), hipFuncAttributeMaxDynamicSharedMemorySize, (int)lds);
        attr = true;
    }
    static_assert(MT == 1, "bwd_grid() assumes 16-row wave tiles in the streamed-weight backward");
    const int grid = bwd_grid(p.C, p.M);
    if (LNB && (int64_t)grid * 2 * p.C > p.part_floats) return -1;
    hipLaunchKernelGGL((convmlp_bwd_kernel<NK, MT, NW, ST, LNB, DG>), dim3(grid), dim3(64 * NW), lds, st, p);
    return LNB ? reduce_ln_partials(p, grid, st) : 0;
}
template <int NK, int MT, int NW>
int launch_bwd(const CmP& p, hipStream_t st) {
    if (p.zin == nullptr) {
        if (p.y) return p.act ? launch_bwd_t<NK, MT, NW, true, true, false>(p, st) : launch_bwd_t<NK, MT, NW, false, true, false>(p, st);
        return p.act ? launch_bwd_t<NK, MT, NW, true, false, false>(p, st) : launch_bwd_t<NK, MT, NW, false, false, false>(p, st);
    }
    if (p.y) return p.act ? launch_bwd_t<NK, MT, NW, true, true, true>(p, st) : launch_bwd_t<NK, MT, NW, false, true, true>(p, st);
    return p.act ? launch_bwd_t<NK, MT, NW, true, false, true>(p, st) : launch_bwd_t<NK, MT, NW, false, false, true>(p, st);
}

}

extern "C" int64_t lnx_convmlp_bwd_ws_floats(int C, int M) {
    if (!lnx_convmlp_supported(LNX_BF16, C) || M <= 0) return 0;
    return (int64_t)bwd_grid(C, M) * 2 * C;
}

extern "C" int lnx_convmlp_supported(int dtype, int C) { return dtype == LNX_BF16 && (C == 32 || C == 64 || C == 96 || C == 128 || C == 192); }

extern "C" int lnx_convmlp_fwd(const lnx_convmlp_args* a, void* stream) {
    LNX_CHECK(a && (a->ln || a->y) && a->w1 && a->w2 && a->b1 && a->b2 && a->gamma && a->x && a->out, "lnx_convmlp_fwd: null operand");
    if (a->y) {
        LNX_CHECK(a->ln_w && a->ln_b && a->ln == nullptr, "lnx_convmlp_fwd: the fused LayerNorm form takes y, ln_w, ln_b and no ln");
        LNX_CHECK((a->mean == nullptr) == (a->ln_out == nullptr) && (a->rstd == nullptr) == (a->ln_out == nullptr) && (a->z == nullptr || a->ln_out != nullptr),
                  "lnx_convmlp_fwd: with y, the outputs ln_out, mean and rstd are written together (what a backward needs) or not at all; z only with them");
    }
    LNX_CHECK(lnx_convmlp_supported(a->dtype, a->C), "lnx_convmlp_fwd: unsupported dtype %d / C %d (bf16, C in {32,64,96,128,192})", a->dtype, a->C);
    LNX_CHECK(a->M > 0, "lnx_convmlp_fwd: empty");
    if (a->rowscale) LNX_CHECK(a->rows_per_sample > 0, "lnx_convmlp_fwd: rowscale needs rows_per_sample");
    CmP p{};
    p.ln = (const unsigned char*)a->ln; p.w1 = (const unsigned char*)a->w1; p.w2 = (const unsigned char*)a->w2;
    p.b1 = a->b1; p.b2 = a->b2; p.gamma = a->gamma; p.rowscale = a->rowscale; p.x = a->x; p.out = a->out; p.z = (unsigned char*)a->z;
    p.M = a->M; p.C = a->C; p.rps = a->rows_per_sample > 0 ? a->rows_per_sample : 1;
    p.y = (const unsigned char*)a->y; p.lnw = a->ln_w; p.lnb = a->ln_b; p.eps = a->ln_eps; p.ln_out = (unsigned char*)a->ln_out; p.mean = a->mean; p.rstd = a->rstd;
    hipStream_t st = (hipStream_t)stream;
    switch (a->C) {
        case 32: launch_fwd_res<1>(p, st); break;
        case 64: launch_fwd_res<2>(p, st); break;
        case 96: launch_fwd_res<3>(p, st); break;
        case 128: if (nw8) launch_fwd<4, 1, 8>(p, st); else launch_fwd<4, 1, 4>(p, st); break;
        case 192: if (nw8) launch_fwd<6, 1, 8>(p, st); else launch_fwd<6, 1, 4>(p, st); break;
    }
    LNX_LAUNCH_CHECK();
    return 0;
}

extern "C" int lnx_convmlp_bwd(const lnx_convmlp_bwd_args* a, void* stream) {
    LNX_CHECK(a && a->g && a->ln && a->w1 && a->w2t && a->w1t && a->b1 && a->gamma && a->dz && a->dln && (a->dgamma || !a->z),
              "lnx_convmlp_bwd: null operand (z may be NULL: dgamma is then not produced here; with z, dgamma is required)");
    LNX_CHECK((a->act == nullptr) == (a->dh == nullptr), "lnx_convmlp_bwd: act and dh must both be given or both be NULL");
    LNX_CHECK(lnx_convmlp_supported(a->dtype, a->C), "lnx_convmlp_bwd: unsupported dtype %d / C %d", a->dtype, a->C);
    LNX_CHECK(a->M > 0, "lnx_convmlp_bwd: empty");
    if (a->rowscale) LNX_CHECK(a->rows_per_sample > 0, "lnx_convmlp_bwd: rowscale needs rows_per_sample");
    if (a->y) LNX_CHECK(a->ln_w && a->mean && a->rstd && a->d_ln_w && a->d_ln_b && a->ws, "lnx_convmlp_bwd: the fused LayerNorm form needs ln_w, mean, rstd, d_ln_w, d_ln_b and ws");
    CmP p{};
    p.y = (const unsigned char*)a->y; p.lnw = a->ln_w; p.mean = const_cast<float*>(a->mean); p.rstd = const_cast<float*>(a->rstd);
    p.part = a->ws; p.part_floats = a->ws_floats; p.dlnw = a->d_ln_w; p.dlnb = a->d_ln_b; p.ln_defer = a->ln_defer;
    p.g = a->g; p.ln = (const unsigned char*)a->ln; p.zin = (const unsigned char*)a->z; p.w1 = (const unsigned char*)a->w1;
    p.w2t = (const unsigned char*)a->w2t; p.w1t = (const unsigned char*)a->w1t; p.b1 = a->b1; p.gamma = a->gamma; p.rowscale = a->rowscale;
    p.act = (unsigned char*)a->act; p.dh = (unsigned char*)a->dh; p.dz = (unsigned char*)a->dz; p.dln = (unsigned char*)a->dln; p.dgamma = a->dgamma;
    p.M = a->M; p.C = a->C; p.rps = a->rows_per_sample > 0 ? a->rows_per_sample : 1;
    p.dz_plain = a->dz_plain != 0;
    hipStream_t st = (hipStream_t)stream;
    int rc = 0;
    switch (a->C) {
        case 32: rc = launch_bwd_res<1, 2>(p, st); break;
        case 64: rc = launch_bwd_res<2, 1>(p, st); break;
        case 96: rc = launch_bwd_res<3, 1>(p, st); break;
        case 128: rc = nw8 ? launch_bwd<4, 1, 8>(p, st) : launch_bwd<4, 1, 4>(p, st); break;
        case 192: rc = nw8 ? launch_bwd<6, 1, 8>(p, st) : launch_bwd<6, 1, 4>(p, st); break;
    }
    LNX_CHECK(rc == 0, "lnx_convmlp_bwd: ws too small for the LayerNorm partial sums (M=%d C=%d ws_floats=%lld)", a->M, a->C, (long long)a->ws_floats);
    LNX_LAUNCH_CHECK();
    return 0;
}
```

Measured before the change: 13320 images/sec.

## Add 2x4 streamed-weight ConvMLP form with 32-wide hidden chunks as default

Templates the streamed-weight ConvMLP forward and backward kernels on the hidden-chunk width and adds a form using 4 waves with two 16-row m-tiles each and 32-wide hidden chunks. This halves per-stage LDS so two workgroups can share a CU at C=192, raising the launch-bounds occupancy hint. The new form becomes the default for the forward pass, while the backward pass keeps the 8-wave path unless the '2x4b' form is selected. Smaller hidden chunks double the loop iterations and barriers, and the MT=2 tiles increase register pressure. Adds a runtime setter for the form and timing stamps for the backward kernel.

New measurement: 13410 images/sec (median of 6 runs). About the same (+0.7%).

```diff
diff --git a/include/lnx.h b/include/lnx.h
--- a/include/lnx.h
+++ b/include/lnx.h
@@ -559,6 +559,7 @@
 } lnx_convmlp_bwd_args;
 int lnx_convmlp_bwd(const lnx_convmlp_bwd_args* args, void* stream);
 int64_t lnx_convmlp_bwd_ws_floats(int C, int M);
+int lnx_convmlp_stream_form(int form);
 
 
 #define LNX_MAX_META 8
diff --git a/linnaeus_amd/_lib.py b/linnaeus_amd/_lib.py
--- a/linnaeus_amd/_lib.py
+++ b/linnaeus_amd/_lib.py
@@ -185,7 +185,7 @@
     "lnx_metrics_table_sizes", "lnx_metrics_update", "lnx_predict",
     "lnx_mix_rows", "lnx_mix_meta",
     "lnx_aug_pointwise", "lnx_aug_saturation", "lnx_aug_rowstat", "lnx_aug_rescale", "lnx_aug_affine", "lnx_aug_stencil", "lnx_erase_rects", "lnx_u8hwc_to_f32chw",
-    "lnx_convmlp_supported", "lnx_convmlp_fwd", "lnx_convmlp_bwd", "lnx_convmlp_bwd_ws_floats",
+    "lnx_convmlp_supported", "lnx_convmlp_fwd", "lnx_convmlp_bwd", "lnx_convmlp_bwd_ws_floats", "lnx_convmlp_stream_form",
     "lnx_plan_create", "lnx_plan_destroy", "lnx_plan_workspace_bytes", "lnx_plan_num_params", "lnx_plan_param_name",
     "lnx_plan_param_numel", "lnx_plan_num_drop_calls", "lnx_plan_logits_numel", "lnx_plan_logits_offset", "lnx_plan_logits_ld",
     "lnx_plan_bind", "lnx_plan_forward", "lnx_plan_backward", "lnx_plan_backward_into", "lnx_plan_segment_params", "lnx_plan_profile_begin", "lnx_plan_profile_end", "lnx_plan_profile_begin_spans", "lnx_plan_profile_end_ex", "lnx_plan_set_wgrad_stream", "lnx_plan_set_meta_stream",
diff --git a/linnaeus_amd/csrc/convmlp.hip b/linnaeus_amd/csrc/convmlp.hip
--- a/linnaeus_amd/csrc/convmlp.hip
+++ b/linnaeus_amd/csrc/convmlp.hip
@@ -55,16 +55,23 @@
     static constexpr int PART = NK * 4096;
     static constexpr int CT = C / 16;
 };
-
-template <int NK, int NW>
+template <int NK, int HN> struct GeoH {
+    static_assert(HN == 64 || HN == 32, "hidden chunk of one or two MFMA k-steps");
+    static constexpr int PART = NK * HN * 64;
+    static constexpr int NT = HN / 16;
+    static constexpr int KS2 = HN / 32;
+};
+
+template <int NK, int NW, int HN = 64>
 __device__ __forceinline__ void dma_nmajor(unsigned char* lds_part, const unsigned char* W, int n0, int wave, int lane) {
     constexpr int C = Geo<NK>::C;
-    constexpr int NINS = 4 * NK;
+    constexpr int RBN = HN / 16;
+    constexpr int NINS = RBN * NK;
     static_assert(NINS % NW == 0, "DMA pieces must divide evenly over the waves");
 #pragma unroll
     for (int t = 0; t < NINS / NW; ++t) {
         const int i = wave + NW * t;
-        const int ks = i >> 2, rb = i & 3;
+        const int ks = i / RBN, rb = i % RBN;
         const int row = 16 * rb + (lane >> 2), u = lane & 3;
         const unsigned char* src = W + ((int64_t)(n0 + row) * C + ks * 32 + ((u ^ key4(row >> 3)) << 3)) * 2;
         __builtin_amdgcn_global_load_lds((const __attribute__((address_space(1))) void*)src,
@@ -72,11 +79,12 @@
     }
 }
 
-template <int NK, int NW>
+template <int NK, int NW, int HN = 64>
 __device__ __forceinline__ void dma_cmajor(unsigned char* lds_part, const unsigned char* W, int n0, int wave, int lane) {
     constexpr int C = Geo<NK>::C;
     constexpr int RB = C / 16;
-    constexpr int NINS = 2 * RB;
+    constexpr int NINS = GeoH<NK, HN>::KS2 * RB;
+    static_assert(NINS % NW == 0, "DMA pieces must divide evenly over the waves");
 #pragma unroll
     for (int t = 0; t < NINS / NW; ++t) {
         const int i = wave + NW * t;
@@ -174,46 +182,52 @@
     }
 }
 
-template <int NK, int MT>
-__device__ __forceinline__ void prod_nmajor_pipe(f32x4_t (&h)[4][MT], uint32_t part_addr, int s, int g, const uint4 (&xf)[MT][NK]) {
+template <int NK, int MT, int HN = 64>
+__device__ __forceinline__ void prod_nmajor_pipe(f32x4_t (&h)[HN / 16][MT], uint32_t part_addr, int s, int g, const uint4 (&xf)[MT][NK]) {
+    constexpr int NT = GeoH<NK, HN>::NT;
+    constexpr int KSTEP = HN * 64;
     const uint32_t unit = (uint32_t)((g ^ key4(s >> 2)) << 4);
     const uint32_t base = part_addr + (uint32_t)((8 * (s >> 2) + (s & 3)) * 64) + unit;
 #pragma unroll
-    for (int nt = 0; nt < 4; ++nt)
+    for (int nt = 0; nt < NT; ++nt)
 #pragma unroll
         for (int mt = 0; mt < MT; ++mt) h[nt][mt] = f32x4_t{0.f, 0.f, 0.f, 0.f};
-    uint4 wf[2][4];
+    uint4 wf[2][NT];
     CM_DS_READ128(wf[0][0], base, 0);
     CM_DS_READ128(wf[0][1], base, 256);
-    CM_DS_READ128(wf[0][2], base, 2048);
-    CM_DS_READ128(wf[0][3], base, 2304);
+    if constexpr (NT == 4) {
+        CM_DS_READ128(wf[0][2], base, 2048);
+        CM_DS_READ128(wf[0][3], base, 2304);
+    }
 #pragma unroll
     for (int ks = 0; ks < NK; ++ks) {
         if (ks + 1 < NK) {
-            const uint32_t a = base + (ks + 1) * 4096;
+            const uint32_t a = base + (ks + 1) * KSTEP;
             CM_DS_READ128(wf[(ks + 1) & 1][0], a, 0);
             CM_DS_READ128(wf[(ks + 1) & 1][1], a, 256);
-            CM_DS_READ128(wf[(ks + 1) & 1][2], a, 2048);
-            CM_DS_READ128(wf[(ks + 1) & 1][3], a, 2304);
-            asm volatile("s_waitcnt lgkmcnt(4)" ::: "memory");
+            if constexpr (NT == 4) {
+                CM_DS_READ128(wf[(ks + 1) & 1][2], a, 2048);
+                CM_DS_READ128(wf[(ks + 1) & 1][3], a, 2304);
+            }
+            asm volatile("s_waitcnt lgkmcnt(%0)" ::"n"(NT) : "memory");
         } else {
             asm volatile("s_waitcnt lgkmcnt(0)" ::: "memory");
         }
         __builtin_amdgcn_sched_barrier(0);
 #pragma unroll
-        for (int nt = 0; nt < 4; ++nt)
+        for (int nt = 0; nt < NT; ++nt)
 #pragma unroll
             for (int mt = 0; mt < MT; ++mt) mfma16(h[nt][mt], wf[ks & 1][nt], xf[mt][ks]);
     }
 }
 
-template <int NK, int MT>
-__device__ __forceinline__ void prod_cmajor_pipe(f32x4_t (&o)[Geo<NK>::CT][MT], uint32_t part_addr, int s, int g, const uint4 (&pf)[MT][2]) {
+template <int NK, int MT, int HN = 64>
+__device__ __forceinline__ void prod_cmajor_pipe(f32x4_t (&o)[Geo<NK>::CT][MT], uint32_t part_addr, int s, int g, const uint4 (&pf)[MT][HN / 32]) {
     constexpr int C = Geo<NK>::C;
     constexpr int CT = Geo<NK>::CT;
     const uint32_t base = part_addr + (uint32_t)(s * 64) + (uint32_t)((g ^ key4(s >> 2)) << 4);
     constexpr int GB = 4;
-    constexpr int NB = 2 * CT / GB;
+    constexpr int NB = GeoH<NK, HN>::KS2 * CT / GB;
     static_assert(CT % GB == 0, "channel tiles must split into batches of 4");
     uint4 wf[2][GB];
 #pragma unroll
@@ -358,25 +372,26 @@
 }
 
 #ifdef CM_STAMP
-__device__ unsigned long long g_cm_stamp[8];
+__device__ unsigned long long g_cm_stamp[16];
 #define CM_T(i) do { __builtin_amdgcn_sched_barrier(0); unsigned long long t_; asm volatile("s_memtime %0\n\ts_waitcnt lgkmcnt(0)" : "=s"(t_) :: "memory"); \
                      __builtin_amdgcn_sched_barrier(0); tsum[i] += t_ - tlast; tlast = t_; } while (0)
 #else
 #define CM_T(i) do { } while (0)
 #endif
 
-template <int NK, int MT, int NW, bool LNF>
-__global__ __launch_bounds__(64 * NW) void convmlp_fwd_kernel(const CmP p) {
+template <int NK, int MT, int NW, bool LNF, int HN = 64>
+__global__ __launch_bounds__(64 * NW, (HN == 32 || NW == 8) ? 2 : 1) void convmlp_fwd_kernel(const CmP p) {
 #ifdef CM_STAMP
     unsigned long long tsum[8] = {0, 0, 0, 0, 0, 0, 0, 0}, tlast;
     asm volatile("s_memtime %0\n\ts_waitcnt lgkmcnt(0)" : "=s"(tlast)::"memory");
 #endif
     constexpr int C = Geo<NK>::C;
     constexpr int CT = Geo<NK>::CT;
-    constexpr int PART = Geo<NK>::PART;
+    constexpr int PART = GeoH<NK, HN>::PART;
+    constexpr int NT = GeoH<NK, HN>::NT;
     constexpr int STAGE = 2 * PART;
-    constexpr int NCH = 4 * C / 64;
-    constexpr int NLD = 8 * NK / NW;
+    constexpr int NCH = 4 * C / HN;
+    constexpr int NLD = 2 * NT * NK / NW;
     extern __shared__ __attribute__((aligned(16))) unsigned char smem[];
     float* b1s = reinterpret_cast<float*>(smem + 3 * STAGE);
 
@@ -421,10 +436,10 @@
         for (int mt = 0; mt < MT; ++mt) o[ct][mt] = f32x4_t{0.f, 0.f, 0.f, 0.f};
 
     __syncthreads();
-    dma_nmajor<NK, NW>(smem, p.w1, 0, wave, lane);
-    dma_cmajor<NK, NW>(smem + PART, p.w2, 0, wave, lane);
-    dma_nmajor<NK, NW>(smem + STAGE, p.w1, 64, wave, lane);
-    dma_cmajor<NK, NW>(smem + STAGE + PART, p.w2, 64, wave, lane);
+    dma_nmajor<NK, NW, HN>(smem, p.w1, 0, wave, lane);
+    dma_cmajor<NK, NW, HN>(smem + PART, p.w2, 0, wave, lane);
+    dma_nmajor<NK, NW, HN>(smem + STAGE, p.w1, HN, wave, lane);
+    dma_cmajor<NK, NW, HN>(smem + STAGE + PART, p.w2, HN, wave, lane);
     CM_T(0);
     for (int j = 0; j < NCH; ++j) {
         const int stg = j % 3;
@@ -435,41 +450,42 @@
         CM_T(2);
         if (j + 2 < NCH) {
             unsigned char* nx = smem + ((j + 2) % 3) * STAGE;
-            dma_nmajor<NK, NW>(nx, p.w1, 64 * (j + 2), wave, lane);
-            dma_cmajor<NK, NW>(nx + PART, p.w2, 64 * (j + 2), wave, lane);
+            dma_nmajor<NK, NW, HN>(nx, p.w1, HN * (j + 2), wave, lane);
+            dma_cmajor<NK, NW, HN>(nx + PART, p.w2, HN * (j + 2), wave, lane);
         }
         const uint32_t st = lds0 + stg * STAGE;
-        f32x4_t h[4][MT];
+        f32x4_t h[NT][MT];
         CM_T(3);
-        prod_nmajor_pipe<NK, MT>(h, st, s, g, xf);
+        prod_nmajor_pipe<NK, MT, HN>(h, st, s, g, xf);
         CM_T(4);
-        uint4 pf[MT][2];
+        uint4 pf[MT][HN / 32];
         {
-            f32x4_t bv[4];
-            const uint32_t ba = lds0 + 3 * STAGE + (uint32_t)((64 * j + 8 * g) * 4);
+            f32x4_t bv[NT];
+            const uint32_t ba = lds0 + 3 * STAGE + (uint32_t)((HN * j + 8 * g) * 4);
             CM_DS_READ128(bv[0], ba, 0);
             CM_DS_READ128(bv[1], ba, 16);
-            CM_DS_READ128(bv[2], ba, 128);
-            CM_DS_READ128(bv[3], ba, 144);
+            if constexpr (NT == 4) {
+                CM_DS_READ128(bv[2], ba, 128);
+                CM_DS_READ128(bv[3], ba, 144);
+            }
             asm volatile("s_waitcnt lgkmcnt(0)" ::: "memory");
             __builtin_amdgcn_sched_barrier(0);
 #pragma unroll
             for (int mt = 0; mt < MT; ++mt)
 #pragma unroll
-                for (int n2 = 0; n2 < 4; n2 += 2) {
+                for (int n2 = 0; n2 < NT; n2 += 2) {
                     f32x4_t hv[2] = {h[n2][mt], h[n2 + 1][mt]};
                     gelu4_bias_n<2>(hv, &bv[n2]);
                     h[n2][mt] = hv[0];
                     h[n2 + 1][mt] = hv[1];
                 }
 #pragma unroll
-            for (int mt = 0; mt < MT; ++mt) {
-                pf[mt][0] = pack8(h[0][mt], h[1][mt]);
-                pf[mt][1] = pack8(h[2][mt], h[3][mt]);
-            }
+            for (int mt = 0; mt < MT; ++mt)
+#pragma unroll
+                for (int k2 = 0; k2 < HN / 32; ++k2) pf[mt][k2] = pack8(h[2 * k2][mt], h[2 * k2 + 1][mt]);
         }
         CM_T(5);
-        prod_cmajor_pipe<NK, MT>(o, st + PART, s, g, pf);
+        prod_cmajor_pipe<NK, MT, HN>(o, st + PART, s, g, pf);
         CM_T(6);
     }
 #pragma unroll
@@ -507,17 +523,22 @@
 #endif
 }
 #ifdef CM_STAMP
-extern "C" int lnx_dbg_convmlp_stamps(unsigned long long* out8) { return (int)hipMemcpyFromSymbol(out8, HIP_SYMBOL(g_cm_stamp), 64); }
+extern "C" int lnx_dbg_convmlp_stamps(unsigned long long* out16) { return (int)hipMemcpyFromSymbol(out16, HIP_SYMBOL(g_cm_stamp), 128); }
 #endif
 
-template <int NK, int MT, int NW, bool ST, bool LNB, bool DG>
+template <int NK, int MT, int NW, bool ST, bool LNB, bool DG, int HN = 64>
 __global__ __launch_bounds__(64 * NW) void convmlp_bwd_kernel(const CmP p) {
+#ifdef CM_STAMP
+    unsigned long long tsum[8] = {0, 0, 0, 0, 0, 0, 0, 0}, tlast;
+    asm volatile("s_memtime %0\n\ts_waitcnt lgkmcnt(0)" : "=s"(tlast)::"memory");
+#endif
     constexpr int C = Geo<NK>::C;
     constexpr int CT = Geo<NK>::CT;
-    constexpr int PART = Geo<NK>::PART;
+    constexpr int PART = GeoH<NK, HN>::PART;
+    constexpr int NT = GeoH<NK, HN>::NT;
     constexpr int STAGE = 3 * PART;
-    constexpr int NCH = 4 * C / 64;
-    constexpr int NLD = 12 * NK / NW;
+    constexpr int NCH = 4 * C / HN;
+    constexpr int NLD = 3 * NT * NK / NW;
     extern __shared__ __attribute__((aligned(16))) unsigned char smem[];
     float* b1s = reinterpret_cast<float*>(smem + 2 * STAGE);
     float* dgs = b1s + 4 * C;
@@ -592,42 +613,52 @@
     for (int ct = 0; ct < CT; ++ct)
 #pragma unroll
         for (int mt = 0; mt < MT; ++mt) dl[ct][mt] = f32x4_t{0.f, 0.f, 0.f, 0.f};
-    LnRow<NK> lrow;
-    if constexpr (LNB) ln_bwd_fetch<NK>(lrow, p, m_base + s, g);
+    LnRow<NK> lrow[MT];
+    if constexpr (LNB) {
+#pragma unroll
+        for (int mt = 0; mt < MT; ++mt) ln_bwd_fetch<NK>(lrow[mt], p, m_base + mt * 16 + s, g);
+    }
 
     __syncthreads();
-    dma_nmajor<NK, NW>(smem, p.w1, 0, wave, lane);
-    dma_nmajor<NK, NW>(smem + PART, p.w2t, 0, wave, lane);
-    dma_cmajor<NK, NW>(smem + 2 * PART, p.w1t, 0, wave, lane);
+    dma_nmajor<NK, NW, HN>(smem, p.w1, 0, wave, lane);
+    dma_nmajor<NK, NW, HN>(smem + PART, p.w2t, 0, wave, lane);
+    dma_cmajor<NK, NW, HN>(smem + 2 * PART, p.w1t, 0, wave, lane);
+    CM_T(0);
     for (int j = 0; j < NCH; ++j) {
         const int stg = j & 1;
         __builtin_amdgcn_s_barrier();
+        CM_T(1);
         if (j + 1 < NCH) {
             unsigned char* nx = smem + (stg ^ 1) * STAGE;
-            dma_nmajor<NK, NW>(nx, p.w1, 64 * (j + 1), wave, lane);
-            dma_nmajor<NK, NW>(nx + PART, p.w2t, 64 * (j + 1), wave, lane);
-            dma_cmajor<NK, NW>(nx + 2 * PART, p.w1t, 64 * (j + 1), wave, lane);
+            dma_nmajor<NK, NW, HN>(nx, p.w1, HN * (j + 1), wave, lane);
+            dma_nmajor<NK, NW, HN>(nx + PART, p.w2t, HN * (j + 1), wave, lane);
+            dma_cmajor<NK, NW, HN>(nx + 2 * PART, p.w1t, HN * (j + 1), wave, lane);
             asm volatile("s_waitcnt vmcnt(%0)" ::"n"(NLD) : "memory");
         } else {
             asm volatile("s_waitcnt vmcnt(0)" ::: "memory");
         }
+        CM_T(2);
         __builtin_amdgcn_s_barrier();
+        CM_T(3);
         const uint32_t st = lds0 + stg * STAGE;
-        f32x4_t h[4][MT], da[4][MT];
-        prod_nmajor_pipe<NK, MT>(h, st, s, g, xf);
-        prod_nmajor_pipe<NK, MT>(da, st + PART, s, g, zf);
-        f32x4_t bv[4];
-        const uint32_t ba = lds0 + 2 * STAGE + (uint32_t)((64 * j + 8 * g) * 4);
+        f32x4_t h[NT][MT], da[NT][MT];
+        prod_nmajor_pipe<NK, MT, HN>(h, st, s, g, xf);
+        prod_nmajor_pipe<NK, MT, HN>(da, st + PART, s, g, zf);
+        CM_T(4);
+        f32x4_t bv[NT];
+        const uint32_t ba = lds0 + 2 * STAGE + (uint32_t)((HN * j + 8 * g) * 4);
         CM_DS_READ128(bv[0], ba, 0);
         CM_DS_READ128(bv[1], ba, 16);
-        CM_DS_READ128(bv[2], ba, 128);
-        CM_DS_READ128(bv[3], ba, 144);
+        if constexpr (NT == 4) {
+            CM_DS_READ128(bv[2], ba, 128);
+            CM_DS_READ128(bv[3], ba, 144);
+        }
         asm volatile("s_waitcnt lgkmcnt(0)" ::: "memory");
         __builtin_amdgcn_sched_barrier(0);
 #pragma unroll
         for (int mt = 0; mt < MT; ++mt)
 #pragma unroll
-            for (int n2 = 0; n2 < 4; n2 += 2) {
+            for (int n2 = 0; n2 < NT; n2 += 2) {
                 f32x4_t hv[2] = {h[n2][mt], h[n2 + 1][mt]}, dv[2] = {da[n2][mt], da[n2 + 1][mt]};
                 gelu4_bias_grad_n<2>(hv, &bv[n2], dv);
                 h[n2][mt] = hv[0];
@@ -635,27 +666,31 @@
                 da[n2][mt] = dv[0];
                 da[n2 + 1][mt] = dv[1];
             }
-        uint4 pa[MT][2], pd[MT][2];
+        uint4 pa[MT][HN / 32], pd[MT][HN / 32];
 #pragma unroll
         for (int mt = 0; mt < MT; ++mt) {
-            pa[mt][0] = pack8(h[0][mt], h[1][mt]);
-            pa[mt][1] = pack8(h[2][mt], h[3][mt]);
-            pd[mt][0] = pack8(da[0][mt], da[1][mt]);
-            pd[mt][1] = pack8(da[2][mt], da[3][mt]);
             const int m = min(m_base + mt * 16 + s, p.M - 1);
+            const int64_t off = ((int64_t)m * (4 * C) + HN * j + 8 * g) * 2;
+#pragma unroll
+            for (int k2 = 0; k2 < HN / 32; ++k2) {
+                pa[mt][k2] = pack8(h[2 * k2][mt], h[2 * k2 + 1][mt]);
+                pd[mt][k2] = pack8(da[2 * k2][mt], da[2 * k2 + 1][mt]);
+            }
             if constexpr (ST) {
-                const int64_t off = ((int64_t)m * (4 * C) + 64 * j + 8 * g) * 2;
-                st16(p.act + off, pa[mt][0]);
-                st16(p.act + off + 64, pa[mt][1]);
-                st16(p.dh + off, pd[mt][0]);
-                st16(p.dh + off + 64, pd[mt][1]);
-            }
-        }
-        prod_cmajor_pipe<NK, MT>(dl, st + 2 * PART, s, g, pd);
+#pragma unroll
+                for (int k2 = 0; k2 < HN / 32; ++k2) st16(p.act + off + 64 * k2, pa[mt][k2]);
+#pragma unroll
+                for (int k2 = 0; k2 < HN / 32; ++k2) st16(p.dh + off + 64 * k2, pd[mt][k2]);
+            }
+        }
+        CM_T(5);
+        prod_cmajor_pipe<NK, MT, HN>(dl, st + 2 * PART, s, g, pd);
+        CM_T(6);
     }
     if constexpr (LNB) {
-        static_assert(MT == 1, "ln_bwd_rows is instantiated per m-tile");
-        ln_bwd_rows<NK, MT, 0>(p, dl, lrow, m_base + s, s, g, lws, dls);
+        static_assert(MT <= 2, "ln_bwd_rows is instantiated per m-tile");
+        ln_bwd_rows<NK, MT, 0>(p, dl, lrow[0], m_base + s, s, g, lws, dls);
+        if constexpr (MT == 2) ln_bwd_rows<NK, MT, 1>(p, dl, lrow[MT - 1], m_base + 16 + s, s, g, lws, dls);
     } else {
 #pragma unroll
         for (int mt = 0; mt < MT; ++mt) {
@@ -675,6 +710,11 @@
         for (int i = threadIdx.x; i < C; i += 64 * NW) atomicAdd(p.dgamma + i, dgs[i]);
     if constexpr (LNB)
         for (int i = threadIdx.x; i < 2 * C; i += 64 * NW) p.part[(int64_t)blockIdx.x * (2 * C) + i] = dls[i];
+    CM_T(7);
+#ifdef CM_STAMP
+    if (blockIdx.x == gridDim.x / 2 && threadIdx.x == 0)
+        for (int i = 0; i < 8; ++i) g_cm_stamp[8 + i] = tsum[i];
+#endif
 }
 
 
@@ -1122,7 +1162,15 @@
     if (w0 < w1) atomicAdd((e < C ? dw : db) + (e < C ? e : e - C), t);
 }
 
-static const bool nw8 = !(getenv("LNX_CM_NW") && atoi(getenv("LNX_CM_NW")) == 4);
+enum { CM_FORM_2X4 = 0, CM_FORM_2X4B = 2, CM_FORM_NW4 = 4, CM_FORM_NW8 = 8 };
+static int form_from_env() {
+    const char* e = getenv("LNX_CM_NW");
+    if (e == nullptr || e[0] == 0) return CM_FORM_2X4;
+    if (e[0] == '2') return e[1] && e[2] && e[3] == 'b' ? CM_FORM_2X4B : CM_FORM_2X4;
+    return atoi(e) == 4 ? CM_FORM_NW4 : CM_FORM_NW8;
+}
+static int cm_form = form_from_env();
+static int stream_rows() { return cm_form == CM_FORM_NW4 ? 64 : 128; }
 
 static int bwd_grid(int C, int M) {
     if (C <= 96) {
@@ -1130,7 +1178,7 @@
         const int grid = cdiv(cdiv(M, rows), 8);
         return grid > 256 ? 256 : grid;
     }
-    return cdiv(M, 16 * (nw8 ? 8 : 4));
+    return cdiv(M, stream_rows());
 }
 
 static int res_room() {
@@ -1195,46 +1243,66 @@
     return p.act ? launch_bwd_res_t<NK, MT, true, false, true>(p, st) : launch_bwd_res_t<NK, MT, false, false, true>(p, st);
 }
 
-template <int NK, int MT, int NW, bool LNF>
+template <int NK, int HN> constexpr size_t fwd_lds() { return 3 * 2 * GeoH<NK, HN>::PART + 4 * Geo<NK>::C * sizeof(float); }
+template <int NK, int HN> constexpr size_t bwd_lds() { return 2 * 3 * GeoH<NK, HN>::PART + 8 * Geo<NK>::C * sizeof(float); }
+static_assert(fwd_lds<6, 32>() <= 80 * 1024 && bwd_lds<6, 32>() <= 80 * 1024, "two co-resident workgroups per CU at C = 192");
+
+template <int NK, int MT, int NW, int HN, bool LNF>
 int launch_fwd_t(const CmP& p, hipStream_t st) {
-    const size_t lds = 3 * 2 * Geo<NK>::PART + 4 * Geo<NK>::C * sizeof(float);
+    const size_t lds = fwd_lds<NK, HN>();
     static bool attr = false;
     if (!attr) {
-        (void)hipFuncSetAttribute(reinterpret_cast<const void*>(&convmlp_fwd_kernel<NK, MT, NW, LNF>), hipFuncAttributeMaxDynamicSharedMemorySize, (int)lds);
+        (void)hipFuncSetAttribute(reinterpret_cast<const void*>(&convmlp_fwd_kernel<NK, MT, NW, LNF, HN>), hipFuncAttributeMaxDynamicSharedMemorySize, (int)lds);
         attr = true;
     }
-    hipLaunchKernelGGL((convmlp_fwd_kernel<NK, MT, NW, LNF>), dim3(cdiv(p.M, 16 * NW * MT)), dim3(64 * NW), lds, st, p);
+    hipLaunchKernelGGL((convmlp_fwd_kernel<NK, MT, NW, LNF, HN>), dim3(cdiv(p.M, 16 * NW * MT)), dim3(64 * NW), lds, st, p);
     return 0;
 }
-template <int NK, int MT, int NW>
+template <int NK, int MT, int NW, int HN>
+int launch_fwd_f(const CmP& p, hipStream_t st) {
+    return p.y ? launch_fwd_t<NK, MT, NW, HN, true>(p, st) : launch_fwd_t<NK, MT, NW, HN, false>(p, st);
+}
+template <int NK>
 int launch_fwd(const CmP& p, hipStream_t st) {
-    return p.y ? launch_fwd_t<NK, MT, NW, true>(p, st) : launch_fwd_t<NK, MT, NW, false>(p, st);
-}
-
-template <int NK, int MT, int NW, bool ST, bool LNB, bool DG>
+    if (cm_form == CM_FORM_2X4 || cm_form == CM_FORM_2X4B) return launch_fwd_f<NK, 2, 4, 32>(p, st);
+    return cm_form == CM_FORM_NW8 ? launch_fwd_f<NK, 1, 8, 64>(p, st) : launch_fwd_f<NK, 1, 4, 64>(p, st);
+}
+
+template <int NK, int MT, int NW, int HN, bool ST, bool LNB, bool DG>
 int launch_bwd_t(const CmP& p, hipStream_t st) {
-    const size_t lds = 2 * 3 * Geo<NK>::PART + 8 * Geo<NK>::C * sizeof(float);
+    const size_t lds = bwd_lds<NK, HN>();
     static bool attr = false;
     if (!attr) {
-        (void)hipFuncSetAttribute(reinterpret_cast<const void*>(&convmlp_bwd_kernel<NK, MT, NW, ST, LNB, DG>), hipFuncAttributeMaxDynamicSharedMemorySize, (int)lds);
+        (void)hipFuncSetAttribute(reinterpret_cast<const void*>(&convmlp_bwd_kernel<NK, MT, NW, ST, LNB, DG, HN>), hipFuncAttributeMaxDynamicSharedMemorySize, (int)lds);
         attr = true;
     }
-    static_assert(MT == 1, "bwd_grid() assumes 16-row wave tiles in the streamed-weight backward");
     const int grid = bwd_grid(p.C, p.M);
+    if (16 * NW * MT != stream_rows()) return -2;
     if (LNB && (int64_t)grid * 2 * p.C > p.part_floats) return -1;
-    hipLaunchKernelGGL((convmlp_bwd_kernel<NK, MT, NW, ST, LNB, DG>), dim3(grid), dim3(64 * NW), lds, st, p);
+    hipLaunchKernelGGL((convmlp_bwd_kernel<NK, MT, NW, ST, LNB, DG, HN>), dim3(grid), dim3(64 * NW), lds, st, p);
     return LNB ? reduce_ln_partials(p, grid, st) : 0;
 }
-template <int NK, int MT, int NW>
+template <int NK, int MT, int NW, int HN>
+int launch_bwd_f(const CmP& p, hipStream_t st) {
+    if (p.zin == nullptr) {
+        if (p.y) return p.act ? launch_bwd_t<NK, MT, NW, HN, true, true, false>(p, st) : launch_bwd_t<NK, MT, NW, HN, false, true, false>(p, st);
+        return p.act ? launch_bwd_t<NK, MT, NW, HN, true, false, false>(p, st) : launch_bwd_t<NK, MT, NW, HN, false, false, false>(p, st);
+    }
+    if (p.y) return p.act ? launch_bwd_t<NK, MT, NW, HN, true, true, true>(p, st) : launch_bwd_t<NK, MT, NW, HN, false, true, true>(p, st);
+    return p.act ? launch_bwd_t<NK, MT, NW, HN, true, false, true>(p, st) : launch_bwd_t<NK, MT, NW, HN, false, false, true>(p, st);
+}
+template <int NK>
 int launch_bwd(const CmP& p, hipStream_t st) {
-    if (p.zin == nullptr) {
-        if (p.y) return p.act ? launch_bwd_t<NK, MT, NW, true, true, false>(p, st) : launch_bwd_t<NK, MT, NW, false, true, false>(p, st);
-        return p.act ? launch_bwd_t<NK, MT, NW, true, false, false>(p, st) : launch_bwd_t<NK, MT, NW, false, false, false>(p, st);
-    }
-    if (p.y) return p.act ? launch_bwd_t<NK, MT, NW, true, true, true>(p, st) : launch_bwd_t<NK, MT, NW, false, true, true>(p, st);
-    return p.act ? launch_bwd_t<NK, MT, NW, true, false, true>(p, st) : launch_bwd_t<NK, MT, NW, false, false, true>(p, st);
-}
-
+    if (cm_form == CM_FORM_2X4B) return launch_bwd_f<NK, 2, 4, 32>(p, st);
+    return cm_form != CM_FORM_NW4 ? launch_bwd_f<NK, 1, 8, 64>(p, st) : launch_bwd_f<NK, 1, 4, 64>(p, st);
+}
+
+}
+
+extern "C" int lnx_convmlp_stream_form(int form) {
+    const int prev = cm_form;
+    if (form == CM_FORM_2X4 || form == CM_FORM_2X4B || form == CM_FORM_NW4 || form == CM_FORM_NW8) cm_form = form;
+    return prev;
 }
 
 extern "C" int64_t lnx_convmlp_bwd_ws_floats(int C, int M) {
@@ -1264,8 +1332,8 @@
         case 32: launch_fwd_res<1>(p, st); break;
         case 64: launch_fwd_res<2>(p, st); break;
         case 96: launch_fwd_res<3>(p, st); break;
-        case 128: if (nw8) launch_fwd<4, 1, 8>(p, st); else launch_fwd<4, 1, 4>(p, st); break;
-        case 192: if (nw8) launch_fwd<6, 1, 8>(p, st); else launch_fwd<6, 1, 4>(p, st); break;
+        case 128: launch_fwd<4>(p, st); break;
+        case 192: launch_fwd<6>(p, st); break;
     }
     LNX_LAUNCH_CHECK();
     return 0;
@@ -1293,9 +1361,10 @@
         case 32: rc = launch_bwd_res<1, 2>(p, st); break;
         case 64: rc = launch_bwd_res<2, 1>(p, st); break;
         case 96: rc = launch_bwd_res<3, 1>(p, st); break;
-        case 128: rc = nw8 ? launch_bwd<4, 1, 8>(p, st) : launch_bwd<4, 1, 4>(p, st); break;
-        case 192: rc = nw8 ? launch_bwd<6, 1, 8>(p, st) : launch_bwd<6, 1, 4>(p, st); break;
-    }
+        case 128: rc = launch_bwd<4>(p, st); break;
+        case 192: rc = launch_bwd<6>(p, st); break;
+    }
+    LNX_CHECK(rc != -2, "lnx_convmlp_bwd: streamed-weight kernel form and launch grid disagree (C=%d)", a->C);
     LNX_CHECK(rc == 0, "lnx_convmlp_bwd: ws too small for the LayerNorm partial sums (M=%d C=%d ws_floats=%lld)", a->M, a->C, (long long)a->ws_floats);
     LNX_LAUNCH_CHECK();
     return 0;
```
